# mikestir/webradio

Measured on AMD Instinct MI355X. Metric: complex Msamples/sec (node), 256-ch DDC+NFM demod, higher is better.
Workload: dtype f32

## Files before the change

### include/webradio_amd.h

```cpp
#ifndef WEBRADIO_AMD_H_
#define WEBRADIO_AMD_H_

#include <stddef.h>
#include <stdint.h>

#ifdef __cplusplus
extern "C" {
#endif

#define WR_ABI_VERSION   6
#define WR_FIR_LENGTH    64
#define WR_TABLE_SIZE    65536

enum wr_status {
	WR_OK = 0,
	WR_ERR_ARG = 1,
	WR_ERR_HIP = 2,
	WR_ERR_STATE = 3,
	WR_ERR_NOMEM = 4,
	WR_ERR_NODEV = 5,
	WR_ERR_RATE = 6
};

enum wr_mode { WR_AM = 0, WR_FM = 1, WR_USB = 2, WR_LSB = 3 };

enum wr_stage {
	WR_STAGE_CHAN_IQ = 1,
	WR_STAGE_DEMOD   = 2,
	WR_STAGE_AUDIO   = 3
};

enum wr_nco {
	WR_NCO_SPLIT = 0,
	WR_NCO_EXACT = 1,
	WR_NCO_ROTATE = 2
};

enum wr_where { WR_HOST = 0, WR_DEVICE = 1 };

typedef struct wr_dev      wr_dev;
typedef struct wr_tuner    wr_tuner;
typedef struct wr_spectrum wr_spectrum;
typedef struct wr_ring     wr_ring;

int         wr_abi_version(void);
const char *wr_last_error(void);
int         wr_device_count(int *count);
enum wr_tunable {
	WR_TUNE_DDC_NG2_MIN_PASSES = 1
};
int         wr_tune(int key, long value, long *previous);

int wr_phase_step(int if_hz, unsigned int input_rate, int *phase_step);
int wr_sin_table(float *table_host);
int wr_lowpass_design(unsigned int passband, unsigned int input_rate,
                      float *coeff_host , unsigned int *maxbin_out);
#define WR_FIR_MAX 1024
#define WR_FIR_FUSED_MAX 256
int wr_lowpass_design_n(unsigned int fir_length, unsigned int passband, unsigned int input_rate,
                        float *coeff_host , unsigned int *maxbin_out);
int wr_spectrum_window(unsigned int fft_size, float *window_host);

int wr_dev_open(wr_dev **dev, int device_index, void *hip_stream);
int wr_dev_close(wr_dev *dev);
int wr_dev_sync(wr_dev *dev);
void *wr_dev_stream(wr_dev *dev);
int wr_dev_malloc(wr_dev *dev, size_t bytes, void **ptr_dev);
int wr_dev_free(wr_dev *dev, void *ptr_dev);
int wr_dev_upload(wr_dev *dev, void *dst_dev, const void *src_host, size_t bytes);
int wr_dev_download(wr_dev *dev, void *dst_host, const void *src_dev, size_t bytes);
int wr_dev_host_register(wr_dev *dev, void *host, size_t bytes);
int wr_dev_host_unregister(wr_dev *dev, void *host);
int wr_dev_upload_async(wr_dev *dev, void *dst_dev, const void *src_host, size_t bytes);
int wr_dev_wait_uploads(wr_dev *dev);
int wr_dev_wait_uploads_but(wr_dev *dev, unsigned int newest);
int wr_dev_upload_ahead(wr_dev *dev, void *dst_dev, const void *src_host, size_t bytes);

int wr_mix(wr_dev *dev, const float *in_dev, float *out_dev, size_t nframes,
           unsigned int *phase_io, int phase_step);

int wr_fir_decimate(wr_dev *dev, const float *in_dev, size_t nframes, unsigned int channels,
                    unsigned int decimation, const float *coeff_host ,
                    float *history_dev, float *out_dev);
int wr_fir_decimate_n(wr_dev *dev, const float *in_dev, size_t nframes, unsigned int channels,
                      unsigned int decimation, unsigned int fir_length, const float *coeff_host ,
                      float *history_dev, float *out_dev);
unsigned long long wr_block_kernel_calls(void);

int wr_demod(wr_dev *dev, int mode, const float *in_dev, size_t nframes,
             float *prev_io , float *out_dev);

int wr_u8_to_f32(wr_dev *dev, const uint8_t *in_dev, float *out_dev, size_t count);
int wr_u8_to_f32_from_host(wr_dev *dev, const uint8_t *in_host_registered, float *out_dev, size_t count);
int wr_stage_windows_from_host(wr_dev *dev, const void *in_host_registered, int is_u8, float *out_dev, size_t nframes,
                               unsigned int period, unsigned int length, size_t tail_frames);

#define WR_MAX_CHANNELS 4096
int wr_tuner_create(wr_tuner **tuner, wr_dev *dev, unsigned int input_rate,
                    unsigned int max_channels, size_t max_block_frames, int nco_mode);
int wr_tuner_destroy(wr_tuner *tuner);

int wr_chan_add(wr_tuner *tuner, int *chan);
int wr_chan_remove(wr_tuner *tuner, int chan);
int wr_chan_count(wr_tuner *tuner, int *count);

int wr_chan_set_if(wr_tuner *tuner, int chan, int if_hz);
int wr_chan_set_filter(wr_tuner *tuner, int chan, int stage, unsigned int passband,
                       unsigned int out_rate);
int wr_chan_set_taps(wr_tuner *tuner, int chan, int stage, const float *coeff_host ,
                     unsigned int decimation);
int wr_chan_set_filter_n(wr_tuner *tuner, int chan, int stage, unsigned int fir_length,
                         unsigned int passband, unsigned int out_rate);
int wr_chan_set_taps_n(wr_tuner *tuner, int chan, int stage, const float *coeff_host ,
                       unsigned int fir_length, unsigned int decimation);
#define WR_FILTER_CHANNEL  0
#define WR_FILTER_AUDIO    1
#define WR_FILTER_CHANNEL2 2
int wr_chan_set_af_gain(wr_tuner *tuner, int chan, float gain_db);
int wr_chan_set_squelch(wr_tuner *tuner, int chan, float threshold_dbfs, int enable);
int wr_chan_set_mode(wr_tuner *tuner, int chan, int mode);
int wr_tuner_keep_stages(wr_tuner *tuner, unsigned int stage_mask);

int wr_chan_get_state(wr_tuner *tuner, int chan, unsigned int *phase, float *prev_iq );
int wr_chan_set_state(wr_tuner *tuner, int chan, unsigned int phase, const float *prev_iq);

int wr_tuner_last_staging(wr_tuner *tuner, int *how);
int wr_tuner_submit(wr_tuner *tuner, const float *iq, size_t nframes, int where);
int wr_tuner_submit_u8(wr_tuner *tuner, const uint8_t *iq_u8, size_t nframes, int where);

int wr_tuner_flush(wr_tuner *tuner);

int wr_chan_fetch(wr_tuner *tuner, int chan, int stage, float *out_host, size_t out_capacity,
                  size_t *count);
int wr_tuner_audio_dev(wr_tuner *tuner, const float **audio_dev, size_t *chan_stride,
                       size_t *frames);
int wr_chan_slot(wr_tuner *tuner, int chan, int *slot);
int wr_tuner_fetch_audio_all(wr_tuner *tuner, float *out_host, size_t out_capacity,
                             size_t *chan_stride, size_t *frames, unsigned int *slots_used);
int wr_tuner_audio_ring(wr_tuner *tuner, unsigned int depth);
int wr_tuner_audio_ring_acquire(wr_tuner *tuner, const float **audio_host, size_t *chan_stride,
                                size_t *frames, unsigned int *slots_used, unsigned long long *seq);
int wr_tuner_audio_ring_release(wr_tuner *tuner);
int wr_tuner_audio_ring_ready(wr_tuner *tuner, int *ready);
int wr_tuner_audio_ring_stats(wr_tuner *tuner, unsigned int *queued, unsigned long long *overruns);
int wr_tuner_submit_count(wr_tuner *tuner, unsigned long long *submits);
int wr_chan_reset_history(wr_tuner *tuner, int chan);
int wr_tuner_seek(wr_tuner *tuner, unsigned long long frame);
int wr_ring_id_bytes(void);
int wr_ring_version(int *version);
int wr_ring_make_id(void *id_host, size_t nbytes);
int wr_ring_create(wr_ring **ring, wr_dev *dev, const void *id_host, size_t nbytes, int rank, int world);
int wr_ring_exchange(wr_ring *ring, const float *send_dev, float *recv_dev, size_t nfloats);
int wr_tuner_mark_launches(wr_tuner *tuner, int enable);
int wr_ring_exchange_after(wr_ring *ring, wr_tuner *tuner, const float *send_dev, float *recv_dev, size_t nfloats);
int wr_ring_wait(wr_ring *ring);
int wr_ring_info(wr_ring *ring, int *rank, int *world, unsigned long long *exchanges);
int wr_ring_destroy(wr_ring *ring);
int wr_tuner_set_audio_scale(wr_tuner *tuner, float scale);

int wr_tuner_set_blocks_per_launch(wr_tuner *tuner, unsigned int nblocks);

#define WR_STREAM_MAX_BLOCKS 512u
int wr_tuner_set_streaming(wr_tuner *tuner, int enable);
int wr_tuner_stream_info(wr_tuner *tuner, int *live, unsigned long long *launches, unsigned long long *blocks);
int wr_tuner_stream_host_blocks(wr_tuner *tuner, unsigned long long *blocks);
int wr_tuner_stream_long_blocks(wr_tuner *tuner, unsigned long long *blocks);

int wr_tuner_profile(wr_tuner *tuner, int enable);
int wr_tuner_profile_read(wr_tuner *tuner, unsigned int *launches, double *mean_ms);

int wr_spectrum_create(wr_spectrum **spec, wr_dev *dev, unsigned int fft_size, unsigned int hop);
int wr_spectrum_destroy(wr_spectrum *spec);
int wr_spectrum_push(wr_spectrum *spec, const float *iq, size_t nframes, int where);
int wr_spectrum_lazy_info(wr_spectrum *spec, unsigned long long *deferred_pushes, unsigned long long *resolves);
int wr_spectrum_get_db(wr_spectrum *spec, float *magnitudes_host );
int wr_spectrum_get_bins(wr_spectrum *spec, float *bins_host );
int wr_spectrum_frames_done(wr_spectrum *spec, unsigned long *frames);
int wr_spectrum_get_waterfall_row(wr_spectrum *spec, unsigned int width, int hold,
                                  float *db_row_host, uint8_t *palette_host);
int wr_spectrum_batch_db(wr_spectrum *spec, const float *iq_dev, size_t nframes_fft,
                         float *db_dev);

#ifdef __cplusplus
}
#endif
#endif
```

### webradio_amd/capi.py

```python
import ctypes as C
import os

_HERE = os.path.dirname(os.path.abspath(__file__))
LIB_PATH = os.path.join(_HERE, "lib", "libwebradio_amd.so")

WR_OK, WR_ERR_ARG, WR_ERR_HIP, WR_ERR_STATE, WR_ERR_NOMEM, WR_ERR_NODEV, WR_ERR_RATE = range(7)
WR_AM, WR_FM, WR_USB, WR_LSB = range(4)
WR_STAGE_CHAN_IQ, WR_STAGE_DEMOD, WR_STAGE_AUDIO = 1, 2, 3
WR_NCO_SPLIT, WR_NCO_EXACT, WR_NCO_ROTATE = 0, 1, 2
WR_HOST, WR_DEVICE = 0, 1
WR_ABI_VERSION = 6
WR_STREAM_MAX_BLOCKS = 512
WR_FIR_LENGTH = 64
WR_TABLE_SIZE = 65536

_fp = C.POINTER(C.c_float)
_vp = C.c_void_p
_u32 = C.c_uint
_sz = C.c_size_t

SIGNATURES = {
    "wr_abi_version": (C.c_int, []),
    "wr_last_error": (C.c_char_p, []),
    "wr_device_count": (C.c_int, [C.POINTER(C.c_int)]),
    "wr_tune": (C.c_int, [C.c_int, C.c_long, C.POINTER(C.c_long)]),
    "wr_phase_step": (C.c_int, [C.c_int, _u32, C.POINTER(C.c_int)]),
    "wr_sin_table": (C.c_int, [_vp]),
    "wr_lowpass_design": (C.c_int, [_u32, _u32, _vp, C.POINTER(_u32)]),
    "wr_lowpass_design_n": (C.c_int, [_u32, _u32, _u32, _vp, C.POINTER(_u32)]),
    "wr_spectrum_window": (C.c_int, [_u32, _vp]),
    "wr_dev_open": (C.c_int, [C.POINTER(_vp), C.c_int, _vp]),
    "wr_dev_close": (C.c_int, [_vp]),
    "wr_dev_sync": (C.c_int, [_vp]),
    "wr_dev_stream": (_vp, [_vp]),
    "wr_dev_malloc": (C.c_int, [_vp, _sz, C.POINTER(_vp)]),
    "wr_dev_free": (C.c_int, [_vp, _vp]),
    "wr_dev_upload": (C.c_int, [_vp, _vp, _vp, _sz]),
    "wr_dev_download": (C.c_int, [_vp, _vp, _vp, _sz]),
    "wr_dev_host_register": (C.c_int, [_vp, _vp, _sz]),
    "wr_dev_host_unregister": (C.c_int, [_vp, _vp]),
    "wr_dev_upload_async": (C.c_int, [_vp, _vp, _vp, _sz]),
    "wr_dev_wait_uploads": (C.c_int, [_vp]),
    "wr_dev_wait_uploads_but": (C.c_int, [_vp, C.c_uint]),
    "wr_dev_upload_ahead": (C.c_int, [_vp, _vp, _vp, _sz]),
    "wr_mix": (C.c_int, [_vp, _vp, _vp, _sz, C.POINTER(_u32), C.c_int]),
    "wr_fir_decimate": (C.c_int, [_vp, _vp, _sz, _u32, _u32, _vp, _vp, _vp]),
    "wr_fir_decimate_n": (C.c_int, [_vp, _vp, _sz, _u32, _u32, _u32, _vp, _vp, _vp]),
    "wr_demod": (C.c_int, [_vp, C.c_int, _vp, _sz, _vp, _vp]),
    "wr_u8_to_f32": (C.c_int, [_vp, _vp, _vp, _sz]),
    "wr_stage_windows_from_host": (C.c_int, [_vp, _vp, C.c_int, _vp, _sz, _u32, _u32, _sz]),
    "wr_u8_to_f32_from_host": (C.c_int, [_vp, _vp, _vp, _sz]),
    "wr_tuner_create": (C.c_int, [C.POINTER(_vp), _vp, _u32, _u32, _sz, C.c_int]),
    "wr_tuner_destroy": (C.c_int, [_vp]),
    "wr_chan_add": (C.c_int, [_vp, C.POINTER(C.c_int)]),
    "wr_chan_remove": (C.c_int, [_vp, C.c_int]),
    "wr_chan_count": (C.c_int, [_vp, C.POINTER(C.c_int)]),
    "wr_chan_set_if": (C.c_int, [_vp, C.c_int, C.c_int]),
    "wr_chan_set_filter": (C.c_int, [_vp, C.c_int, C.c_int, _u32, _u32]),
    "wr_chan_set_taps": (C.c_int, [_vp, C.c_int, C.c_int, _vp, _u32]),
    "wr_chan_set_filter_n": (C.c_int, [_vp, C.c_int, C.c_int, _u32, _u32, _u32]),
    "wr_chan_set_taps_n": (C.c_int, [_vp, C.c_int, C.c_int, _vp, _u32, _u32]),
    "wr_chan_set_mode": (C.c_int, [_vp, C.c_int, C.c_int]),
    "wr_chan_set_af_gain": (C.c_int, [_vp, C.c_int, C.c_float]),
    "wr_chan_set_squelch": (C.c_int, [_vp, C.c_int, C.c_float, C.c_int]),
    "wr_tuner_keep_stages": (C.c_int, [_vp, _u32]),
    "wr_tuner_flush": (C.c_int, [_vp]),
    "wr_tuner_set_blocks_per_launch": (C.c_int, [_vp, _u32]),
    "wr_tuner_set_streaming": (C.c_int, [_vp, C.c_int]),
    "wr_tuner_stream_info": (C.c_int, [_vp, C.POINTER(C.c_int), C.POINTER(C.c_ulonglong), C.POINTER(C.c_ulonglong)]),
    "wr_tuner_stream_host_blocks": (C.c_int, [_vp, C.POINTER(C.c_ulonglong)]),
    "wr_tuner_stream_long_blocks": (C.c_int, [_vp, C.POINTER(C.c_ulonglong)]),
    "wr_tuner_seek": (C.c_int, [_vp, C.c_ulonglong]),
    "wr_tuner_audio_ring": (C.c_int, [_vp, _u32]),
    "wr_tuner_audio_ring_acquire": (C.c_int, [_vp, C.POINTER(C.POINTER(C.c_float)), C.POINTER(C.c_size_t),
                                              C.POINTER(C.c_size_t), C.POINTER(_u32), C.POINTER(C.c_ulonglong)]),
    "wr_tuner_audio_ring_release": (C.c_int, [_vp]),
    "wr_tuner_audio_ring_ready": (C.c_int, [_vp, C.POINTER(C.c_int)]),
    "wr_tuner_audio_ring_stats": (C.c_int, [_vp, C.POINTER(_u32), C.POINTER(C.c_ulonglong)]),
    "wr_tuner_submit_count": (C.c_int, [_vp, C.POINTER(C.c_ulonglong)]),
    "wr_chan_get_state": (C.c_int, [_vp, C.c_int, C.POINTER(_u32), _vp]),
    "wr_chan_set_state": (C.c_int, [_vp, C.c_int, _u32, _vp]),
    "wr_tuner_submit": (C.c_int, [_vp, _vp, _sz, C.c_int]),
    "wr_tuner_last_staging": (C.c_int, [_vp, C.POINTER(C.c_int)]),
    "wr_block_kernel_calls": (C.c_ulonglong, []),
    "wr_tuner_submit_u8": (C.c_int, [_vp, _vp, _sz, C.c_int]),
    "wr_chan_fetch": (C.c_int, [_vp, C.c_int, C.c_int, _vp, _sz, C.POINTER(_sz)]),
    "wr_tuner_audio_dev": (C.c_int, [_vp, C.POINTER(_vp), C.POINTER(_sz), C.POINTER(_sz)]),
    "wr_chan_slot": (C.c_int, [_vp, C.c_int, C.POINTER(C.c_int)]),
    "wr_tuner_fetch_audio_all": (C.c_int, [_vp, _vp, _sz, C.POINTER(_sz), C.POINTER(_sz), C.POINTER(_u32)]),
    "wr_chan_reset_history": (C.c_int, [_vp, C.c_int]),
    "wr_ring_id_bytes": (C.c_int, []),
    "wr_ring_version": (C.c_int, [C.POINTER(C.c_int)]),
    "wr_ring_make_id": (C.c_int, [_vp, _sz]),
    "wr_ring_create": (C.c_int, [C.POINTER(_vp), _vp, _vp, _sz, C.c_int, C.c_int]),
    "wr_ring_exchange": (C.c_int, [_vp, _vp, _vp, _sz]),
    "wr_ring_exchange_after": (C.c_int, [_vp, _vp, _vp, _vp, _sz]),
    "wr_tuner_mark_launches": (C.c_int, [_vp, C.c_int]),
    "wr_ring_wait": (C.c_int, [_vp]),
    "wr_ring_info": (C.c_int, [_vp, C.POINTER(C.c_int), C.POINTER(C.c_int), C.POINTER(C.c_ulonglong)]),
    "wr_ring_destroy": (C.c_int, [_vp]),
    "wr_tuner_set_audio_scale": (C.c_int, [_vp, C.c_float]),
    "wr_spectrum_get_waterfall_row": (C.c_int, [_vp, _u32, C.c_int, _vp, _vp]),
    "wr_tuner_profile": (C.c_int, [_vp, C.c_int]),
    "wr_tuner_profile_read": (C.c_int, [_vp, C.POINTER(_u32), C.POINTER(C.c_double)]),
    "wr_spectrum_create": (C.c_int, [C.POINTER(_vp), _vp, _u32, _u32]),
    "wr_spectrum_destroy": (C.c_int, [_vp]),
    "wr_spectrum_push": (C.c_int, [_vp, _vp, _sz, C.c_int]),
    "wr_spectrum_lazy_info": (C.c_int, [_vp, C.POINTER(C.c_ulonglong), C.POINTER(C.c_ulonglong)]),
    "wr_spectrum_get_db": (C.c_int, [_vp, _vp]),
    "wr_spectrum_get_bins": (C.c_int, [_vp, _vp]),
    "wr_spectrum_frames_done": (C.c_int, [_vp, C.POINTER(C.c_ulong)]),
    "wr_spectrum_batch_db": (C.c_int, [_vp, _vp, _sz, _vp]),
}


class WrError(RuntimeError):
    def __init__(self, code, msg):
        super().__init__("webradio_amd error %d: %s" % (code, msg))
        self.code = code


_lib = None


def load():
    global _lib
    if _lib is not None:
        return _lib
    if not os.path.exists(LIB_PATH):
        raise RuntimeError(
            "%s is missing: build it with `python -c 'import __graft_entry__ as g; g.build()'` "
            "(there is no CPU fallback)" % LIB_PATH)
    try:
        import torch
    except Exception:
        pass
    lib = C.CDLL(LIB_PATH, mode=C.RTLD_GLOBAL)
    for name, (res, args) in SIGNATURES.items():
        fn = getattr(lib, name)
        fn.restype = res
        fn.argtypes = args
    _lib = lib
    return lib


def check(rc):
    if rc != WR_OK:
        raise WrError(rc, load().wr_last_error().decode(errors="replace"))
    return rc


def ptr(x):
    if x is None:
        return None
    if isinstance(x, int):
        return C.c_void_p(x)
    if hasattr(x, "data_ptr"):
        return C.c_void_p(x.data_ptr())
    return C.c_void_p(x.ctypes.data)
```

### webradio_amd/csrc/wr_capi_internal.h

```cpp
#ifndef WR_CAPI_INTERNAL_H
#define WR_CAPI_INTERNAL_H

#include "wr_internal.h"

#include <cstdarg>
#include <cstdio>
#include <cstdlib>
#include <cstring>
#include <new>
#include <atomic>
#include <chrono>
#include <map>
#include <mutex>
#include <vector>

#define HIP_TRY(expr)                                                                    \
	do {                                                                                 \
		hipError_t e_ = (expr);                                                          \
		if (e_ != hipSuccess)                                                            \
			return wrc_fail(WR_ERR_HIP, "%s: %s (%s:%d)", #expr, hipGetErrorString(e_),  \
			                __FILE__, __LINE__);                                         \
	} while (0)


#define WR_UPLOAD_RING 4

struct wr_dev {
	int device;
	hipStream_t stream;
	bool own_stream;
	int num_cus;
	float *table;
	float *table_turn;
	float *turn_host;
	float *hi_cs, *lo_cs;
	float *scratch;
	size_t scratch_floats;
	float *coeff;
	std::mutex *scratch_lock;
	hipEvent_t upload_ev[WR_UPLOAD_RING];
	std::atomic<unsigned long long> uploads_issued, uploads_done;
	std::mutex *upload_lock;
	hipStream_t up_stream;
	hipStream_t lazy_stream = nullptr;
	hipEvent_t up_tail[WR_UPLOAD_RING], up_done;
	void *up_out[WR_UPLOAD_RING];
	unsigned long long up_calls;
	uint8_t *up_raw[2];
	size_t up_raw_cap[2];
	std::map<void *, size_t> *registered;
	wr_tuner *streaming = nullptr;
	unsigned long long reg_gen = 1;
};
#define SCRATCH_GUARD(d) std::lock_guard<std::mutex> scratch_guard_(*(d)->scratch_lock)

struct Chan {
	bool in_use;
	int if_hz;
	unsigned int stepL;
	unsigned int phaseL;
	int mode;
	bool have[3];
	float taps[3][WR_FIR_LENGTH];
	unsigned int len1;
	float taps_long[WR_FIR_FUSED_MAX];
	unsigned int len2, len1b;
	float taps_long2[WR_FIR_FUSED_MAX], taps_long1b[WR_FIR_FUSED_MAX];
	unsigned int decim[3];
	float gain;
	float squelch;
	bool cs_hist_reset;
	int group;
	int slot;
	float prev_iq[2];
	bool prev_dirty;
	bool phase_dirty;
	bool dem_hist_reset;
};

struct Group {
	unsigned int d1, d2;
	unsigned int d1b = 0;
	unsigned int l1 = WR_FIR_LENGTH;
	unsigned int l2 = WR_FIR_LENGTH;
	unsigned int l1b = WR_FIR_LENGTH;
	int p2 = 0;
	bool use_gain = false, use_squelch = false;
	unsigned int slots;
	size_t k1max, k2max;
	WrGroupDev dev;
	int audio_cur = 0;
	int parity;
	int last_parity;
	bool last_demod_kept = false;
	bool post_pending = false;
	WrPostArgs post_args;
	bool seek_pending = false;
	unsigned long long seek_frame = 0;
	float *z_hist = nullptr, *z_prev = nullptr, *z_dem = nullptr;
	bool pend_direct = false;
	unsigned long long pend_seq = 0;
	size_t pend_k2 = 0;
	unsigned int pend_slots = 0;
	int sp;
	int cb;
	int last_cb;
	std::vector<int> owner;
	bool dirty;
	bool uniform_taps;
	unsigned long long uniform_mask = 0;
	unsigned long long uniform2_mask = 0;
	unsigned long long fewsets_mask = 0;
	unsigned char nsets[64] = {0};
	bool one_filter = false;
	bool long_uniform = false;
	bool long_one = false;
	size_t last_k1, last_k2;
	int active;
};

struct wr_tuner {
	wr_dev *dev;
	unsigned int input_rate;
	unsigned int max_channels;
	size_t max_block_frames;
	int nco_mode;
	unsigned int keep_mask;
	std::vector<Chan> chans;
	std::vector<Group *> groups;
	float *in_stage;
	int last_staging = 0;
	const void *probe_ptr = nullptr;
	unsigned long long probe_gen = 0;
	unsigned int probe_left = 0;
	float *in_hist[2];
	int in_par;
	bool submitted;
	float audio_scale;
	bool profiling;
	unsigned int prof_stride;
	unsigned int prof_tick;
	std::vector<unsigned int> ev_span;
	bool mark_launches = false;
	hipEvent_t launch_ev[4] = {nullptr, nullptr, nullptr, nullptr};
	unsigned long long launches_marked = 0;
	std::vector<hipEvent_t> ev;
	size_t ev_used;
	double prof_ms;
	unsigned int prof_n;
	struct RingSlot {
		float *host = nullptr;
		size_t cap = 0;
		hipEvent_t done = nullptr;
		size_t stride = 0, frames = 0;
		unsigned int slots = 0;
		unsigned long long seq = 0;
		unsigned int stream_wait = 0;
		unsigned long long stream_gen = 0;
	};
	std::vector<RingSlot> ring;
	unsigned int ring_head = 0, ring_count = 0;
	bool ring_held = false;
	unsigned long long ring_overruns = 0;
	unsigned long long submit_seq = 0;
	bool defer_post = true;
	unsigned int coalesce = 1;
	const float *held_base = nullptr;
	size_t held_frames = 0, held_each = 0;
	unsigned int held_count = 0;
	std::mutex ring_lock;
	struct Stream {
		bool enabled = false;
		bool host_bytes = false;
		bool live = false;
		bool unchecked = false;
		WrStreamCtl *ctl = nullptr;
		WrStreamDesc *desc = nullptr;
		WrStreamDev *sdev = nullptr;
		float *ring = nullptr;
		size_t ring_floats = 0;
		Group *g = nullptr;
		unsigned int count = 0;
		size_t nframes = 0;
		bool u8 = false;
		int parity0 = 0;
		size_t k1 = 0, k2 = 0;
		unsigned long long gen = 0;
		unsigned long long blocks = 0;
		std::chrono::steady_clock::time_point last_bell;
		const float *last_iq = nullptr;
		uint8_t *raw[4] = {nullptr, nullptr, nullptr, nullptr};
		size_t raw_cap = 0;
		unsigned long long raw_next = 0;
		unsigned long long raw_gen[4] = {0, 0, 0, 0};
		unsigned int raw_idx[4] = {0, 0, 0, 0};
		hipEvent_t raw_ev = nullptr;
		bool ext = false;
		bool up_pending = false;
		unsigned long long host_blocks = 0;
		unsigned long long long_blocks = 0;
	} stream;
};

struct wr_spectrum {
	wr_dev *dev;
	unsigned int n, hop;
	WrFftPlan plan;
	float *stage;
	size_t stage_cap;
	size_t pending;
	float *bins;
	unsigned long frames_done;
	bool deferred = false;
	float *keep_host = nullptr;
	size_t keep_cap = 0;
	size_t def_off = 0, def_keep = 0;
	size_t def_rest = 0;
	hipEvent_t def_ev = nullptr;
	unsigned long long deferred_pushes = 0, resolves = 0;
};


int        wrc_dev_bind(wr_dev *d);
int        wrc_dev_settle_stream(wr_dev *d);
hipError_t wrc_dev_stream_sync(wr_dev *d);
int        wrc_dev_scratch(wr_dev *d, size_t floats);
void      *wrc_host_mapped(const void *host, hipError_t *why = nullptr);
int        wrc_upload_mark_locked(wr_dev *d, hipStream_t st);
int        wrc_upload_mark(wr_dev *d, hipStream_t st);
int        wrc_dev_up_stream(wr_dev *d);

unsigned int  wrc_group_slots_used(const Group *g);
WrTunerLaunch wrc_group_launch(const wr_tuner *t, const Group *g, const float *cur, const uint8_t *cur_u8, size_t nframes);
Group        *wrc_single_group(wr_tuner *t, bool *several = nullptr);
int           wrc_group_upload(wr_tuner *t, Group *g);
int           wrc_settle_held(wr_tuner *t);
int           wrc_tuner_launch_held(wr_tuner *t);
int           wrc_tuner_flush(wr_tuner *t);
int           wrc_tuner_quiesce(wr_tuner *t);
int           wrc_tuner_submit_now(wr_tuner *t, const void *iq, size_t nframes, int where, bool u8);
void          wrc_advance_phases(wr_tuner *t, unsigned long long frames);
int           wrc_prof_pair_begin(wr_tuner *t, void **ev_start, void **ev_stop);
void          wrc_prof_pair_stamped(wr_tuner *t);

int  wrc_stream_close(wr_tuner *t);
int  wrc_stream_check(wr_tuner *t);
void wrc_stream_free(wr_tuner *t);
bool wrc_stream_follows(const wr_tuner *t, size_t nframes, int where, bool u8);
int  wrc_stream_bell(wr_tuner *t, const void *iq, bool behind_upload);
int  wrc_stream_open(wr_tuner *t, const void *iq, size_t nframes, bool u8, bool *took);
int  wrc_stream_host_u8(wr_tuner *t, const uint8_t *bytes, size_t nframes, bool *took);

float *wrc_ring_reserve(wr_tuner *t, Group *g, size_t k2, unsigned int used);
int    wrc_ring_push(wr_tuner *t, Group *g, unsigned long long seq, size_t k2, unsigned int used, bool direct);
float *wrc_stream_ring_entry(wr_tuner *t, Group *g, unsigned long long seq, size_t k2, unsigned int used, unsigned int idx);

#define DEV_SETTLE(d_) do { if (int rc_ = wrc_dev_settle_stream(d_)) return rc_; } while (0)
#define TUNER_SYNC_CHECKED(t_) do { HIP_TRY(wrc_dev_stream_sync((t_)->dev)); if (int rc_ = wrc_stream_check(t_)) return rc_; } while (0)

#define WR_STREAM_IDLE_MS   500
#define WR_STREAM_STALE_MS  100
#define WR_STREAM_WAIT_MS  2000
#define WR_STREAM_HOST_MIN_BYTES (16u << 10)

#endif
```

### webradio_amd/csrc/wr_internal.h

```cpp
#ifndef WR_INTERNAL_H_
#define WR_INTERNAL_H_

#include <hip/hip_runtime.h>
#include <stddef.h>
#include <stdint.h>

#include "webradio_amd.h"

#define WR_HIST      (WR_FIR_LENGTH - 1)
#define WR_LANES     64
#define WR_SPLIT_N   256
#define WR_MAX_DEVICES 64
#define WR_TAPSETS   4

int         wrc_fail(int code, const char *fmt, ...) __attribute__((format(printf, 2, 3)));
int         wrc_dev_index(const wr_dev *dev);
hipStream_t wrc_dev_stream(const wr_dev *dev);
int         wrc_tuner_launch_mark(wr_tuner *t, hipEvent_t *ev);

void     wrd_sin_table(float *table);
void     wrd_sin_table_rounded(float *table);
int      wrd_phase_step(int if_hz, unsigned int input_rate);
unsigned wrd_lowpass_maxbin(unsigned int fir_length, unsigned int passband, unsigned int input_rate);
void     wrd_lowpass_design(unsigned int fir_length, unsigned int passband, unsigned int input_rate, float *coeff);
void     wrd_spectrum_window(unsigned int n, float *window);
void     wrd_split_tables(float *hi_cs , float *lo_cs );
void     wrd_twiddles(unsigned int n, float *tw );

struct WrGroupDev {
	unsigned int *phase[2];
	unsigned int *step;
	float        *hist_cs[2];
	float        *hist_lo[2];
	int          *flags;
	int          *mode;
	float        *taps1;
	float        *taps2;
	float        *taps2u;
	float        *rot;
	float        *taps1u;
	int          *tapsel;
	float        *taps1b;
	float        *iq2_hist[2];
	float        *chan_iq2[2];
	float        *taps1L;
	float        *mixhist[2];
	float        *gain;
	float        *squelch;
	float        *prev_iq[2];
	float        *chan_iq[2];
	float        *dem[2];
	float        *audio;
	float        *audio_set[4];
	unsigned int  l2 = 64, l1b = 64;
};

struct WrTunerLaunch {
	const float *cur;
	const uint8_t *cur_u8;
	const float *hist;
	float       *hist_next;
	int          parity;
	int          sp;
	int          cb;
	size_t       nframes;
	unsigned int d1, d2;
	unsigned int slots;
	unsigned int slots_used;
	size_t       k1, k2;
	size_t       k2max;
	int          nco_mode;
	float        audio_scale;
	int          use_gain, use_squelch;
	unsigned long long uniform_mask;
	unsigned long long uniform2_mask;
	unsigned long long fewsets_mask;
	unsigned char nsets[64];
	int          one_filter;
	void        *ev_start, *ev_stop;
	bool         seeking = false;
	unsigned int seek_lo = 0;
};

hipError_t wrk_mix(hipStream_t st, const float *in, float *out, size_t nframes,
                   unsigned int phase, int step, const float *table_dev);
hipError_t wrk_fir(hipStream_t st, const float *in, size_t nframes, unsigned int channels,
                   unsigned int decim, unsigned int fir_length, const float *coeff_dev, const float *hist_dev,
                   float *out);
hipError_t wrk_hist_update(hipStream_t st, const float *in, size_t nframes, unsigned int channels,
                           unsigned int fir_length, float *hist_dev, float *scratch_dev);
hipError_t wrk_demod(hipStream_t st, int mode, const float *in, size_t nframes, float prev_i,
                     float prev_q, float *out);
hipError_t wrk_u8_to_f32(hipStream_t st, const uint8_t *in, float *out, size_t count);
hipError_t wrk_stage_windows(hipStream_t st, const void *src_mapped, bool u8, float *dst, size_t nframes, unsigned int period,
                             unsigned int len, size_t tail_frames);

struct WrPostArgs {
	const float *chan_iq;
	unsigned int k1, slots;
	const int   *mode;
	const float *prev_iq;
	float       *prev_next;
	const float *dem_hist;
	float       *dem_hist_next;
	size_t       k2;
	unsigned int tiles;
	unsigned int run;
	unsigned int ntiles;
	const float *taps2;
	const float *taps2u;
	unsigned long long uni2;
	float       *audio;
	size_t       k2max;
	float        scale;
	unsigned int d2;
	unsigned int groups;
	const float *gain;
	const float *squelch;
	float       *audio_host;
	size_t       host_stride;
	unsigned int nseg = 1;
	const float *chan_prev = nullptr;
};
long wrk_tune_ng2_min_passes(long value, bool set);
hipError_t wrk_tuner_ddc(hipStream_t st, const WrTunerLaunch &L, const WrGroupDev &G,
                         const float *table_dev, const float *hi_dev, const float *lo_dev,
                         int num_cus, const WrPostArgs *post = nullptr, bool *post_taken = nullptr);
hipError_t wrk_tuner_ddc_long(hipStream_t st, const WrTunerLaunch &L, const WrGroupDev &G, unsigned int len,
                              const float *table_dev, int num_cus, bool rotate, bool rotate_one_filter, const float *hi_dev,
                              const float *lo_dev, const WrPostArgs *post = nullptr, bool *post_taken = nullptr);
hipError_t wrk_tuner_demod(hipStream_t st, const WrTunerLaunch &L, const WrGroupDev &G);
hipError_t wrk_tuner_iq2(hipStream_t st, const WrGroupDev &G, unsigned int slots, unsigned int slots_used,
                         size_t k1a, unsigned int d1b, int cb, int p2);
hipError_t wrk_tuner_audio(hipStream_t st, const WrTunerLaunch &L, const WrGroupDev &G);
WrPostArgs wrk_post_args(const WrTunerLaunch &L, const WrGroupDev &G);
hipError_t wrk_tuner_post(hipStream_t st, const WrTunerLaunch &L, const WrGroupDev &G);
hipError_t wrk_tuner_post_args(hipStream_t st, const WrPostArgs &A);
bool wrk_tuner_post_supported(unsigned int d2);
hipError_t wrk_input_hist(hipStream_t st, const float *cur, const uint8_t *cur_u8, size_t nframes,
                          const float *hist, float *hist_next);
hipError_t wrk_seek(hipStream_t st, const WrGroupDev &G, unsigned int slots, int sp, int parity, int p2,
                    unsigned long long frame);
hipError_t wrk_gather_rows(hipStream_t st, const float *src, size_t rows, size_t row_stride_floats,
                           size_t col_offset_floats, unsigned int width_floats, float *dst);

#define WR_STREAM_MAXJ   WR_STREAM_MAX_BLOCKS
#define WR_STREAM_RING   6u
struct WrStreamDesc {
	unsigned long long cur;
	unsigned long long audio_host;
	unsigned int count;
	unsigned int pad;
};
struct WrStreamCtl {
	volatile unsigned int ready;
	volatile unsigned int stop;
	volatile unsigned int pad0[14];
	volatile unsigned int done;
	volatile unsigned int final_blocks;
	volatile unsigned int err;
	volatile unsigned int self_closed;
	volatile unsigned int long_blocks;
	volatile unsigned int pad1[11];
};
#define WR_STREAM_SHARDS 16u
struct WrStreamDev {
	unsigned int ready, stop;
	unsigned long long beat;
	unsigned int ready_up;
	unsigned int pad0[27];
	unsigned long long progress;
	unsigned int drain_from;
	unsigned int pad1[29];
	unsigned int post_done[WR_STREAM_MAXJ];
	unsigned int post_fine[WR_STREAM_MAXJ];
	unsigned int post_ticket[WR_STREAM_MAXJ];
	unsigned int ddc_done[WR_STREAM_MAXJ][WR_STREAM_SHARDS][32];
	WrStreamDesc desc[WR_STREAM_MAXJ];
	unsigned long long cur[WR_STREAM_MAXJ + 1u];
};
struct WrStreamArgs {
	WrStreamCtl        *ctl;
	const WrStreamDesc *desc_host;
	WrStreamDev        *sdev;
	unsigned long long  idle_ticks;
	unsigned long long  wait_ticks;
	unsigned int        n_ddc, n_post;
	unsigned long long *tl;
	unsigned long long  cur0, audio0;
	unsigned long long  nframes;
	unsigned int        k1, d1, is_u8;
	unsigned int        ext;
	unsigned int        slots, groups;
	unsigned long long  gmap0, gmap1;
	unsigned int        kslow;
	unsigned int        kmax;
	const float        *hist;
	float              *hist_next;
	const unsigned int *phase, *step;
	unsigned int       *phase_next;
	const float        *hist_cs, *hist_lo;
	float              *hist_cs_next, *hist_lo_next;
	const int          *flags;
	const float        *taps1, *rot, *taps1u;
	const int          *tapsel;
	const float        *table, *hi_cs, *lo_cs;
	float              *ring;
	float              *audio_bufs[4];
	WrPostArgs          post;
	unsigned int        drain_run, drain_ntiles;
	const float        *prev_iq[2];
	float              *dem[2];
	int                 parity0;
	unsigned int        one_filter;
};
#define WR_STREAM_ERR_WAIT   1u
hipError_t wrk_stream_geometry(unsigned int d2, unsigned int groups, unsigned int kmax, bool one_filter, unsigned int nseg,
                               int num_cus, unsigned int *n_ddc, unsigned int *n_post);
hipError_t wrk_tuner_stream(hipStream_t st, const WrStreamArgs &A, void *ev_start, void *ev_stop);

struct WrFftPlan {
	unsigned int n;
	unsigned int n1, n2;
	float *tw_n;
	float *tw_sub;
	float *window;
	float *window_p1;
	float *work;
	size_t work_frames;
};
hipError_t wrk_fft_frames(hipStream_t st, const WrFftPlan &P, const float *iq, size_t hop,
                          size_t nframes_fft, float *bins_out , float *db_out );

hipError_t wrk_bins_to_db(hipStream_t st, const float *bins, unsigned int n, float *db);
hipError_t wrk_waterfall_row(hipStream_t st, const float *bins, unsigned int n, unsigned int width, int hold,
                             float *db_row, uint8_t *palette);

#endif
```

### webradio_amd/csrc/wr_kernels.hip

```cpp
#include "wr_internal.h"

#include <atomic>
#include <cstdlib>
#include <type_traits>

#include <hip/hip_ext.h>

typedef float v2f __attribute__((ext_vector_type(2)));
typedef __attribute__((address_space(3))) v2f lds_v2f;
typedef float v4f __attribute__((ext_vector_type(4)));
typedef __attribute__((address_space(3))) v4f lds_v4f;

#define PHASE_FLAG_ACTIVE   1

#define WR_CONSTANT __attribute__((address_space(4)))

#ifdef DDC_TIMELINE
#define TL_SLOTS 12
__device__ unsigned long long g_ddc_tl[16384 * TL_SLOTS];
extern "C" int wr_debug_timeline(unsigned long long *out, size_t n)
{
	return (int)hipMemcpyFromSymbol(out, HIP_SYMBOL(g_ddc_tl), n * sizeof(unsigned long long));
}
__device__ unsigned long long g_ddc_rt[16384 * 2];
// ... 49 lines not shown
		out[n] = y;
	}
}

__global__ void __launch_bounds__(256)
k_fir(const float *__restrict__ in, size_t outfloats, unsigned int channels, unsigned int decim,
      unsigned int L, const float *__restrict__ coeff, const float *__restrict__ hist, float *__restrict__ out)
{
	__shared__ float taps[WR_FIR_MAX];
	for (unsigned int j = threadIdx.x; j < L; j += blockDim.x)
		taps[j] = coeff[j];
	__syncthreads();
	const unsigned int nh = L - 1u;
	size_t stride = (size_t)gridDim.x * blockDim.x;
	for (size_t o = (size_t)blockIdx.x * blockDim.x + threadIdx.x; o < outfloats; o += stride) {
		size_t k = o / channels;
		unsigned int c = (unsigned int)(o - k * channels);
		size_t first = k * decim;
		float acc = 0.0f;
		for (unsigned int j = 0; j < L; ++j) {
			size_t f = first + j;
			float x = (f < nh) ? hist[f * channels + c] : in[(f - nh) * channels + c];
			acc = acc + taps[L - 1u - j] * x;
		}
		out[o] = acc;
	}
}

__global__ void k_hist_build(const float *__restrict__ in, size_t nframes, unsigned int channels, unsigned int nh,
                             const float *__restrict__ hist, float *__restrict__ scratch)
{
	unsigned int total = nh * channels;
	for (unsigned int e = blockIdx.x * blockDim.x + threadIdx.x; e < total; e += gridDim.x * blockDim.x) {
		size_t f = nframes + e / channels;
		unsigned int c = e % channels;
		scratch[e] = (f < nh) ? hist[f * channels + c] : in[(f - nh) * channels + c];
	}
}

__global__ void k_copy_f32(const float *__restrict__ src, float *__restrict__ dst, size_t n)
{
	size_t stride = (size_t)gridDim.x * blockDim.x;
	for (size_t i = (size_t)blockIdx.x * blockDim.x + threadIdx.x; i < n; i += stride)
		dst[i] = src[i];
}

__device__ __forceinline__ float fm_angle_cycles(float y, float x)
{
	const float ax = __builtin_fabsf(x), ay = __builtin_fabsf(y);
	const float mx = __builtin_fmaxf(ax, ay), mn = __builtin_fminf(ax, ay);
	const float sc = (mx < 0x1p-100f) ? 0x1p100f : 1.0f;
	const float r = (mx == 0.0f) ? 0.0f : (mn * sc) * __builtin_amdgcn_rcpf(mx * sc);
	const float t = r * r;
	float p = 0.002456712769344449f;
	p = __builtin_fmaf(p, t, -0.014401308260858059f);
	p = __builtin_fmaf(p, t, 0.03978113830089569f);
	p = __builtin_fmaf(p, t, -0.07234849780797958f);
	p = __builtin_fmaf(p, t, 0.1049894168972969f);
	p = __builtin_fmaf(p, t, -0.14161227643489838f);
	p = __builtin_fmaf(p, t, 0.19985906779766083f);
	p = __builtin_fmaf(p, t, -0.33332598209381104f);
	p = __builtin_fmaf(p, t, 0.9999998807907104f);
	float c = (p * r) * 0.15915494309189533577f;
	if (ay > ax)
		c = 0.25f - c;
	if (__builtin_signbitf(x))
		c = 0.5f - c;
	return __builtin_copysignf(c, y);
}

__device__ __forceinline__ float demod_one(int mode, float i, float q, float pi_, float pq_)
{
	switch (mode) {
	case WR_AM:
		return (float)sqrt((double)(i * i + q * q));
	case WR_FM: {
		float ii = i * pi_ + q * pq_;
		float qq = q * pi_ - i * pq_;
		return fm_angle_cycles(ii, qq);
	}
	case WR_USB:
		return i + q;
	default:
		return i - q;
	}
}

__global__ void __launch_bounds__(256)
k_demod(int mode, const float2 *__restrict__ in, size_t nframes, float prev_i, float prev_q,
        float *__restrict__ out)
{
	size_t stride = (size_t)gridDim.x * blockDim.x;
	for (size_t n = (size_t)blockIdx.x * blockDim.x + threadIdx.x; n < nframes; n += stride) {
		float2 z = in[n];
		float2 p = n ? in[n - 1] : make_float2(prev_i, prev_q);
		out[n] = demod_one(mode, z.x, z.y, p.x, p.y);
	}
}

__global__ void k_u8_to_f32(const uint8_t *__restrict__ in, float *__restrict__ out, size_t n)
{
	size_t stride = (size_t)gridDim.x * blockDim.x;
	for (size_t i = (size_t)blockIdx.x * blockDim.x + threadIdx.x; i < n; i += stride)
		out[i] = ((float)in[i] - 128.0f) / 128.0f;
}

#define U8_X16_WGS 128u
__global__ void __launch_bounds__(256) k_u8_to_f32_x16(const uint4 *__restrict__ in, float4 *__restrict__ out, size_t n16)
{
	const size_t stride = (size_t)gridDim.x * blockDim.x;
	for (size_t i0 = (size_t)blockIdx.x * blockDim.x + threadIdx.x; i0 < n16; i0 += 4 * stride) {
		uint4 v[4];
#pragma unroll
		for (int u = 0; u < 4; ++u)
			if (i0 + u * stride < n16)
				v[u] = in[i0 + u * stride];
#pragma unroll
		for (int u = 0; u < 4; ++u) {
			const size_t i = i0 + u * stride;
			if (i >= n16)
				break;
			const unsigned int w[4] = {v[u].x, v[u].y, v[u].z, v[u].w};
#pragma unroll
			for (int q = 0; q < 4; ++q) {
				float4 o;
				o.x = ((float)(w[q] & 255u) - 128.0f) / 128.0f;
				o.y = ((float)((w[q] >> 8) & 255u) - 128.0f) / 128.0f;
				o.z = ((float)((w[q] >> 16) & 255u) - 128.0f) / 128.0f;
				o.w = ((float)(w[q] >> 24) - 128.0f) / 128.0f;
				out[4 * i + q] = o;
			}
		}
	}
}


template <int NCO>
__device__ __forceinline__ v2f nco(unsigned int P, const float *__restrict__ table,
                                   const v2f *hi_l, const v2f *lo_l)
{
	if (NCO == WR_NCO_EXACT) {
		v2f cs;
		cs.y = table[P >> 16];
		cs.x = table[(P + 0x40000000u) >> 16];
		return cs;
	} else {
		constexpr unsigned int SH = (NCO == WR_NCO_SPLIT) ? 5u : 0u;
		const v2f a = hi_l[(P >> 24) << SH];
		const v2f b = lo_l[((P >> 16) & 255u) << SH];
		const v2f rot = {-a.y, a.x};
		return __builtin_elementwise_fma(rot, b.yy, a * b.xx);
	}
}

template <int NCO>
__device__ __forceinline__ void mac(v2f xs, v2f cs, float hj, v2f &acc)
{
	if (NCO == WR_NCO_EXACT) {
		const float mi = xs.x * cs.x + xs.y * cs.y;
		const float mq = xs.y * cs.x - xs.x * cs.y;
		float ti, tq;
		asm("v_mul_f32 %0, %1, %2" : "=v"(ti) : "v"(hj), "v"(mi));
		asm("v_mul_f32 %0, %1, %2" : "=v"(tq) : "v"(hj), "v"(mq));
		acc.x = acc.x + ti;
		acc.y = acc.y + tq;
	} else {
		const v2f xr = {xs.y, -xs.x};
		const v2f m = __builtin_elementwise_fma(xr, cs.yy, xs * cs.xx);
		asm("v_fmac_f32 %0, %1, %2" : "+v"(acc.x) : "v"(hj), "v"(m.x));
		asm("v_fmac_f32 %0, %1, %2" : "+v"(acc.y) : "v"(hj), "v"(m.y));
	}
}

__device__ __forceinline__ unsigned int rot_index(unsigned int p0, unsigned int st, unsigned int m)
{
	const unsigned int P = p0 + m * st;
	return (st >> 16) + (((P & 0xFFFFu) < (st & 0xFFFFu)) ? 1u : 0u);
}

__device__ __forceinline__ v2f rot_into(unsigned int p0, unsigned int st, unsigned int m,
                                        const float *__restrict__ table)
{
	const unsigned int idx = rot_index(p0, st, m);
	v2f r;
	r.y = table[idx & 0xFFFFu];
	r.x = table[(idx + 16384u) & 0xFFFFu];
	return r;
}

__device__ __forceinline__ void horner_step(v2f &A, float rc, float rs, v2f u)
{
	const float tr = __builtin_fmaf(-A.y, rs, u.x);
	const float ti = __builtin_fmaf(A.x, rs, u.y);
	const float ar = __builtin_fmaf(A.x, rc, tr);
	const float ai = __builtin_fmaf(A.y, rc, ti);
	A.x = ar;
	A.y = ai;
}

__device__ __forceinline__ void horner_close(v2f &y, v2f A, v2f cs)
{
	const float yr = __builtin_fmaf(A.y, cs.y, __builtin_fmaf(A.x, cs.x, y.x));
	const float yi = __builtin_fmaf(-A.x, cs.y, __builtin_fmaf(A.y, cs.x, y.y));
	y.x = yr;
	y.y = yi;
}

__device__ __forceinline__ void wave_prio(unsigned int level)
{
	if (level >= 3u)
		__builtin_amdgcn_s_setprio(3);
	else if (level == 2u)
		__builtin_amdgcn_s_setprio(2);
	else if (level == 1u)
		__builtin_amdgcn_s_setprio(1);
	else
		__builtin_amdgcn_s_setprio(0);
}

__device__ __forceinline__ void rot_tables_to_lds(v2f *lds, const float2 *hi_cs, const float2 *lo_cs)
{
	for (unsigned int e = threadIdx.x; e < WR_SPLIT_N; e += blockDim.x) {
		const float2 hv = hi_cs[e], lv = lo_cs[e];
		lds[e] = (v2f){hv.x, hv.y};
		lds[WR_SPLIT_N + e] = (v2f){lv.x, lv.y};
	}
	__syncthreads();
}

#define ROT_SEG 64
#define ROT_Q   (WR_FIR_LENGTH / ROT_SEG)
#define SLOW_CH 4

__device__ __forceinline__ void gather_split(unsigned int P, unsigned int &ah, unsigned int &al,
                                             v2f &a, v2f &b)
{
	asm("v_mov_b32_sdwa %0, %1 dst_sel:BYTE_1 dst_unused:UNUSED_PRESERVE src0_sel:BYTE_3"
	    : "+v"(ah) : "v"(P));
	asm("v_mov_b32_sdwa %0, %1 dst_sel:BYTE_1 dst_unused:UNUSED_PRESERVE src0_sel:BYTE_2"
	    : "+v"(al) : "v"(P));
	a = *(const lds_v2f *)(uintptr_t)ah;
	b = *(const lds_v2f *)(uintptr_t)al;
}

__device__ __forceinline__ float2 input_frame(const float2 *__restrict__ cur, const uchar2 *__restrict__ cur_u8,
                                              size_t n)
{
	if (cur_u8) {
		const uchar2 b = cur_u8[n];
		return make_float2(((float)b.x - 128.0f) / 128.0f, ((float)b.y - 128.0f) / 128.0f);
	}
	return cur[n];
}

#define POST_TK 16u
#define POST_B 4u
#define POST_LB 5u
#define POST_THREADS 512u
__device__ __forceinline__ float audio_out(float v, const float *__restrict__ gain, const float *__restrict__ squelch,
                                           const float2 *__restrict__ chan_iq, unsigned int slots, unsigned int so,
                                           size_t k, unsigned int d2, float scale)
{
	if (squelch) {
		const float thr = squelch[so];
		if (thr > 0.0f) {
			float p = 0.0f;
			for (unsigned int i = 0; i < d2; ++i) {
				const float2 z = chan_iq[(k * d2 + i) * slots + so];
				p = p + (z.x * z.x + z.y * z.y);
			}
			if (p / (float)d2 < thr)
				v = 0.0f;
		}
	}
	if (gain) {
		const float gn = gain[so];
		if (gn != 1.0f)
			v = v * gn;
	}
	return (scale == 1.0f) ? v : v * scale;
}

__device__ __forceinline__ float post_row(const float2 *__restrict__ chan_iq, unsigned int k1, unsigned int slots,
                                          unsigned int s, int m, const float2 *__restrict__ prev_iq,
                                          const float *__restrict__ dem_hist, size_t rr,
                                          const float2 *__restrict__ chan_prev = nullptr, unsigned int hist = WR_HIST)
{
	if (rr < hist) {
		if (!chan_prev)
			return dem_hist[rr * slots + s];
		const size_t kp = (size_t)k1 - hist + rr;
		const float2 z = chan_prev[kp * slots + s];
		const float2 zp = chan_prev[(kp - 1u) * slots + s];
		return demod_one(m, z.x, z.y, zp.x, zp.y);
	}
	const size_t kk = rr - hist;
	if (kk >= k1)
		return 0.0f;
	const float2 z = chan_iq[kk * slots + s];
	const float2 zp = kk ? chan_iq[(kk - 1u) * slots + s] : chan_prev ? chan_prev[((size_t)k1 - 1u) * slots + s] : prev_iq[s];
	return demod_one(m, z.x, z.y, zp.x, zp.y);
}

template <unsigned int D2, bool HREGS, unsigned int NSEG = 1u>
__device__ __forceinline__ void post_role(const WrPostArgs &A, unsigned int bx, unsigned int g,
                                          float *stage, float *tile, int *modes)
{
	constexpr unsigned int HIST = WR_FIR_LENGTH * NSEG - 1u;
	constexpr unsigned int NEED = (POST_TK - 1u) * D2 + WR_FIR_LENGTH * NSEG;
	constexpr unsigned int NROW = POST_THREADS / 64u;
	static_assert(NSEG == 1u || !HREGS, "the segmented filter reads its taps when their turn comes (measured at C2, 128 / 256 taps: "
	                                    "61 / 83 us per block; a segment's 64 taps fetched into registers first: 64 / 94)");
	const float2 *__restrict__ chan_iq = (const float2 *)A.chan_iq;
	const float2 *__restrict__ prev_iq = (const float2 *)A.prev_iq;
	const float2 *__restrict__ chan_prev = (const float2 *)A.chan_prev;
	const float *__restrict__ dem_hist = A.dem_hist;
	const float *__restrict__ taps2 = A.taps2;
	const unsigned int k1 = A.k1, slots = A.slots;
	const unsigned int lane = threadIdx.x & 63u;
	const unsigned int row = threadIdx.x >> 6;
	const unsigned int s = g * 64u + lane;
	const int m = A.mode[s];

	if (bx == A.ntiles) {
		if (m < 0)
			return;
		const size_t first = k1;
#pragma unroll
		for (unsigned int r = row; r < HIST; r += NROW)
			A.dem_hist_next[(size_t)r * slots + s] = post_row(chan_iq, k1, slots, s, m, prev_iq, dem_hist, first + r, chan_prev, HIST);
		if (row == 0)
			((float2 *)A.prev_next)[s] = k1 ? chan_iq[(size_t)(k1 - 1u) * slots + s] : prev_iq[s];
		return;
	}

	TLP(0);
	float h[HREGS ? WR_FIR_LENGTH : 1];
	if (HREGS && row < POST_TK / POST_B) {
#pragma unroll
		for (int j = 0; j < (HREGS ? WR_FIR_LENGTH : 1); ++j)
			h[j] = taps2[(size_t)j * slots + s];
	}
	if (row == 0)
		modes[lane] = m;
	constexpr unsigned int FRESH = POST_TK * D2;
	constexpr unsigned int CARRY = NEED - FRESH;
	constexpr unsigned int CARRY_PER = (CARRY * 64u + POST_THREADS - 1u) / POST_THREADS;
	for (unsigned int tt = 0; tt < A.run; ++tt) {
		const unsigned int tl = bx * A.run + tt;
		if (tl >= A.tiles)
			break;
		const size_t kbase = (size_t)tl * POST_TK;
		const size_t r0 = kbase * D2;
		unsigned int first = 0;
		if (tt) {
			float keep[CARRY_PER];
#pragma unroll
			for (unsigned int i = 0; i < CARRY_PER; ++i) {
				const unsigned int e = threadIdx.x + i * POST_THREADS;
				keep[i] = (e < CARRY * 64u) ? stage[FRESH * 64u + e] : 0.0f;
			}
			__syncthreads();
#pragma unroll
			for (unsigned int i = 0; i < CARRY_PER; ++i) {
				const unsigned int e = threadIdx.x + i * POST_THREADS;
				if (e < CARRY * 64u)
					stage[e] = keep[i];
			}
			first = CARRY;
		}
		{
			const unsigned int per = (NEED - first + NROW - 1u) / NROW;
			const unsigned int beg = first + row * per;
			const unsigned int end = (beg + per < NEED) ? beg + per : NEED;
			if (r0 > HIST && r0 + NEED <= (size_t)k1 + HIST) {
				const float2 *__restrict__ src = chan_iq + (r0 - HIST) * slots + s;
				for (unsigned int r = beg; r < end; r += POST_LB) {
					float2 z[POST_LB + 1u];
					z[0] = src[((size_t)r - 1u) * slots];
#pragma unroll
					for (unsigned int i = 0; i < POST_LB; ++i) {
						const unsigned int ri = (r + i < end) ? r + i : end - 1u;
						z[i + 1u] = src[(size_t)ri * slots];
					}
#pragma unroll
					for (unsigned int i = 0; i < POST_LB; ++i)
						if (r + i < end)
							stage[(r + i) * 64u + lane] = (m >= 0) ? demod_one(m, z[i + 1u].x, z[i + 1u].y, z[i].x, z[i].y) : 0.0f;
				}
			} else {
				float2 zp = make_float2(0.0f, 0.0f);
				if (m >= 0 && beg < end) {
					const size_t rr = r0 + beg;
					if (rr == HIST)
						zp = chan_prev ? chan_prev[((size_t)k1 - 1u) * slots + s] : prev_iq[s];
					else if (rr > HIST && rr - HIST - 1u < k1)
						zp = chan_iq[(rr - HIST - 1u) * slots + s];
					else if (rr < HIST && chan_prev)
						zp = chan_prev[((size_t)k1 - HIST - 1u + rr) * slots + s];
				}
#pragma unroll 6
				for (unsigned int r = beg; r < end; ++r) {
					const size_t rr = r0 + r;
					float v = 0.0f;
					if (m >= 0) {
						if (rr < HIST && chan_prev) {
							const float2 z = chan_prev[((size_t)k1 - HIST + rr) * slots + s];
							v = demod_one(m, z.x, z.y, zp.x, zp.y);
							zp = z;
						} else if (rr < HIST) {
							v = dem_hist[rr * slots + s];
							if (rr + 1u == HIST)
								zp = prev_iq[s];
						} else if (rr - HIST < k1) {
							const float2 z = chan_iq[(rr - HIST) * slots + s];
							v = demod_one(m, z.x, z.y, zp.x, zp.y);
							zp = z;
						}
					}
					stage[r * 64u + lane] = v;
				}
			}
		}
		__syncthreads();
		TLP(1);
		if (row < POST_TK / POST_B) {
			float acc[POST_B];
#pragma unroll
			for (unsigned int o = 0; o < POST_B; ++o)
				acc[o] = 0.0f;
			if (HREGS) {
				const float *x = stage + (row * POST_B * D2) * 64u + lane;
#pragma unroll
				for (unsigned int r = 0; r < (POST_B - 1u) * D2 + WR_FIR_LENGTH; ++r) {
					const float xv = x[r * 64u];
#pragma unroll
					for (unsigned int o = 0; o < POST_B; ++o) {
						if (r >= o * D2 && r - o * D2 < WR_FIR_LENGTH)
							acc[o] = acc[o] + h[HREGS ? WR_FIR_LENGTH - 1u - (r - o * D2) : 0] * xv;
					}
				}
			} else {
#pragma unroll 1
			for (unsigned int seg = 0; seg < NSEG; ++seg) {
				const float *x = stage + (row * POST_B * D2 + seg * WR_FIR_LENGTH) * 64u + lane;
				const unsigned int tap0 = (NSEG - 1u - seg) * WR_FIR_LENGTH;
				if (g < 64u && ((A.uni2 >> g) & 1ull)) {
					const WR_CONSTANT float *tu = (const WR_CONSTANT float *)(A.taps2u + (size_t)g * (WR_FIR_LENGTH * NSEG) + tap0);
#pragma unroll
					for (int j = WR_FIR_LENGTH - 1; j >= 0; --j) {
						const float hj = tu[j];
#pragma unroll
						for (unsigned int o = 0; o < POST_B; ++o)
							acc[o] = acc[o] + hj * x[(o * D2 + (WR_FIR_LENGTH - 1u - (unsigned int)j)) * 64u];
					}
				} else {
#pragma unroll 16
					for (int j = WR_FIR_LENGTH - 1; j >= 0; --j) {
						const float hj = taps2[((size_t)tap0 + j) * slots + s];
#pragma unroll
						for (unsigned int o = 0; o < POST_B; ++o)
							acc[o] = acc[o] + hj * x[(o * D2 + (WR_FIR_LENGTH - 1u - (unsigned int)j)) * 64u];
					}
				}
			}
			}
#pragma unroll
			for (unsigned int o = 0; o < POST_B; ++o)
				tile[(row * POST_B + o) * 65u + lane] = acc[o];
		}
		__syncthreads();
		TLP(2);
		for (unsigned int e = threadIdx.x; e < 64u * POST_TK; e += POST_THREADS) {
			const unsigned int sl = e / POST_TK, kk = e - sl * POST_TK;
			const unsigned int so = g * 64u + sl;
			const size_t k = kbase + kk;
			if (k < A.k2 && modes[sl] >= 0) {
				const float v = audio_out(tile[kk * 65u + sl], A.gain, A.squelch, chan_iq, slots, so, k, D2, A.scale);
				A.audio[(size_t)so * A.k2max + k] = v;
				if (A.audio_host)
					A.audio_host[(size_t)so * A.host_stride + k] = v;
			} else if (k < A.k2 && A.audio_host) {
				A.audio_host[(size_t)so * A.host_stride + k] = 0.0f;
			}
		}
		TLP(3);
	}
}

template <unsigned int D2, unsigned int NSEG = 1u>
__global__ void __launch_bounds__(POST_THREADS)
k_tuner_post(WrPostArgs A)
{
	constexpr unsigned int NEED = (POST_TK - 1u) * D2 + WR_FIR_LENGTH * NSEG;
	if constexpr (NSEG == 1u) {
		__shared__ float stage[NEED * 64u];
		__shared__ float tile[POST_TK * 65u];
		__shared__ int modes[64];
		post_role<D2, NSEG == 1u, NSEG>(A, blockIdx.x, blockIdx.y, stage, tile, modes);
	} else {
		extern __shared__ float post_lds[];
		float *stage = post_lds;
		float *tile = stage + NEED * 64u;
		int *modes = (int *)(tile + POST_TK * 65u);
		post_role<D2, NSEG == 1u, NSEG>(A, blockIdx.x, blockIdx.y, stage, tile, modes);
	}
}

#define DDC_TABLE_BYTES   (2u * WR_SPLIT_N * 32u * 8u)
#define DDC_WAVES         16u
#define DDC_ROTATE_WAVES      8u
#define DDC_ROTATE_WGS_PER_CU 4u
#define DDC_LDS_BYTES     (DDC_TABLE_BYTES + DDC_WAVES * 2u * 512u)
#define DDC_DEAL_WAYS 2u

#define DDC_PARAMS \
	const float2 *__restrict__ cur, const uchar2 *__restrict__ cur_u8, const float2 *__restrict__ hist, \
	float2 *__restrict__ hist_next, size_t nframes, size_t k1, unsigned int d1, unsigned int slots, unsigned int groups, \
	const unsigned int *__restrict__ phase, const unsigned int *__restrict__ step, \
	const float2 *__restrict__ hist_cs, const int *__restrict__ flags, \
	unsigned int *__restrict__ phase_next, float2 *__restrict__ hist_cs_next, \
	const float2 *__restrict__ hist_lo, float2 *__restrict__ hist_lo_next, \
	const float *__restrict__ taps1, const float4 *__restrict__ rot, const float *__restrict__ taps1u, \
	const int *__restrict__ tapsel, unsigned int kmax, float2 *__restrict__ chan_iq, \
	const float *__restrict__ table, const float2 *__restrict__ hi_cs, const float2 *__restrict__ lo_cs, \
	unsigned int n_ddc, const WrPostArgs &post, unsigned long long gmap0, unsigned long long gmap1, int whole, \
	unsigned int kslow, unsigned int n_bnd, unsigned int seek_on, unsigned int seek_lo
#define DDC_PASS \
	cur, cur_u8, hist, hist_next, nframes, k1, d1, slots, groups, phase, step, hist_cs, flags, phase_next, hist_cs_next, \
	hist_lo, hist_lo_next, taps1, rot, taps1u, tapsel, kmax, chan_iq, table, hi_cs, lo_cs, n_ddc, post, gmap0, gmap1, \
	whole, kslow, n_bnd, seek_on, seek_lo
#define DDC_PHASE(s_) (seek_on ? step[s_] * seek_lo : phase[s_])
#define DDC_ROLE_ALL      0
#define DDC_ROLE_BOUNDARY 1
#define DDC_ROLE_ROLL     2

template <int NCO, bool UTAPS, unsigned int PD2>
__device__ __forceinline__ void
ddc_body(DDC_PARAMS, v2f *lds, const int role)
{
	if (PD2 != 0u && role != DDC_ROLE_ROLL && blockIdx.x >= n_ddc + n_bnd) {
		wave_prio(3u);
		constexpr unsigned int NEED = (POST_TK - 1u) * (PD2 ? PD2 : 1u) + WR_FIR_LENGTH;
		const unsigned int idx = blockIdx.x - n_ddc - n_bnd;
		if (threadIdx.x >= POST_THREADS)
			return;
		float *stage = (float *)lds;
		post_role<(PD2 ? PD2 : 1u), false>(post, idx % (post.ntiles + 1u), idx / (post.ntiles + 1u), stage,
		                                    stage + NEED * 64u, (int *)(stage + NEED * 64u + POST_TK * 65u));
		return;
	}
	const unsigned int lane = threadIdx.x & 63u;
	const unsigned int wave = __builtin_amdgcn_readfirstlane(threadIdx.x >> 6);
	const unsigned int waves_per_wg = blockDim.x >> 6;
	const unsigned int wid = blockIdx.x * waves_per_wg + wave;
	TL(0);
	wave_prio(3u);

	if (NCO == WR_NCO_SPLIT) {
		for (unsigned int e = threadIdx.x; e < WR_SPLIT_N * 32u; e += blockDim.x) {
			const float2 hv = hi_cs[e >> 5], lv = lo_cs[e >> 5];
			lds[e] = (v2f){hv.x, hv.y};
			lds[WR_SPLIT_N * 32u + e] = (v2f){lv.x, lv.y};
		}
		__syncthreads();
	} else if (NCO == WR_NCO_ROTATE) {
		rot_tables_to_lds(lds, hi_cs, lo_cs);
	}
	const v2f *hi_l = (NCO == WR_NCO_ROTATE) ? lds : lds + (lane & 31u);
	const v2f *lo_l = (NCO == WR_NCO_ROTATE) ? lds + WR_SPLIT_N : lds + WR_SPLIT_N * 32u + (lane & 31u);
	const unsigned int a_hi = (unsigned int)(uintptr_t)hi_l;
	const unsigned int a_lo = (unsigned int)(uintptr_t)lo_l;
	const unsigned int nset = UTAPS ? kmax : 1u;
	v2f *win = lds + (NCO == WR_NCO_SPLIT ? DDC_TABLE_BYTES / 8u : NCO == WR_NCO_ROTATE ? 2u * WR_SPLIT_N : 0u)
	           + wave * (128u * nset);

	if (whole && role != DDC_ROLE_ROLL && blockIdx.x == 0 && wave == 0 && lane < WR_HIST) {
		const size_t f = nframes + lane;
		hist_next[lane] = (f < WR_HIST) ? hist[f] : input_frame(cur, cur_u8, f - WR_HIST);
	}

	const unsigned int k1u = (unsigned int)k1;
	const unsigned int nwaves = n_ddc * waves_per_wg;
	TL(1);
	constexpr bool LTAPS = (NCO == WR_NCO_ROTATE) && !UTAPS;
	unsigned int wpg = LTAPS ? (n_ddc / groups) * waves_per_wg : nwaves / groups;
	const bool bnd = role == DDC_ROLE_BOUNDARY;
	const unsigned int ub = bnd ? (blockIdx.x - n_ddc) * waves_per_wg + wave : 0u;
	const unsigned int gl = bnd ? ub % groups : LTAPS ? blockIdx.x % groups : wid % groups;
	const unsigned int g = (unsigned int)(((gl < 8u ? gmap0 : gmap1) >> ((gl & 7u) * 8u)) & 255u);
	unsigned int k = bnd ? ub / groups : LTAPS ? (blockIdx.x / groups) * waves_per_wg + wave : wid / groups;
	if (role == DDC_ROLE_ROLL) {
		k = k1u;
	} else if (bnd) {
		if (k >= kslow)
			k = k1u;
		wpg = k1u;
	} else if (k >= wpg) {
		k = k1u;
	} else if (!LTAPS) {
		const unsigned int r = k % DDC_DEAL_WAYS, q = k / DDC_DEAL_WAYS;
		const unsigned int fl_ = wpg / DDC_DEAL_WAYS, rem = wpg % DDC_DEAL_WAYS;
		k = r * fl_ + (r < rem ? r : rem) + q;
	}
	const float *ltaps = (const float *)(lds + (NCO == WR_NCO_ROTATE ? 2u * WR_SPLIT_N : 0u) + waves_per_wg * 128u * nset);
	if (LTAPS) {
		float *lt = (float *)(lds + 2u * WR_SPLIT_N + waves_per_wg * 128u * nset);
		for (unsigned int e = threadIdx.x; e < WR_FIR_LENGTH * 64u; e += blockDim.x)
			lt[e] = taps1[(size_t)(e >> 6) * slots + g * 64u + (e & 63u)];
		__syncthreads();
	}

	float h[(UTAPS || LTAPS) ? 1 : WR_FIR_LENGTH];
	float hlane[UTAPS ? WR_TAPSETS : 1];
	unsigned int mysel = 0;
#pragma unroll
	for (int q = 0; q < (UTAPS ? WR_TAPSETS : 1); ++q)
		hlane[q] = 0.0f;
	unsigned int p0 = 0, st = 0;
	int fl = 0;
	unsigned int buf = 0;
	v2f rot0 = {1.0f, 0.0f}, rot1 = {1.0f, 0.0f};

	auto window_sample = [&](unsigned int kk) -> float2 {
		const long long n = (long long)kk * d1 - WR_HIST + lane;
		return (n >= 0) ? input_frame(cur, cur_u8, (size_t)n) : hist[WR_HIST + n];
	};
	float2 xnext = make_float2(0.0f, 0.0f);
	float2 xnext2 = make_float2(0.0f, 0.0f);
	const unsigned int s = g * 64u + lane;
	if (k < k1u) {
		{
			p0 = DDC_PHASE(s);
			st = step[s];
			fl = flags[s];
			if (NCO == WR_NCO_ROTATE) {
				const float4 r = rot[s];
				rot0 = (v2f){r.x, r.y};
				rot1 = (v2f){r.z, r.w};
			}
			if (UTAPS) {
				mysel = (unsigned int)tapsel[s];
#pragma unroll
				for (int q = 0; q < (UTAPS ? WR_TAPSETS : 1); ++q)
					if ((unsigned int)q < nset)
						hlane[q] = taps1u[((size_t)g * WR_TAPSETS + q) * 64u + lane];
			} else {
#pragma unroll
				for (int j = 0; j < ((UTAPS || LTAPS) ? 1 : WR_FIR_LENGTH); ++j)
					h[j] = taps1[(size_t)j * slots + s];
			}
		}
		xnext = window_sample(k);
		if (k + wpg < k1u)
			xnext2 = window_sample(k + wpg);
	}

	TL(2);
	unsigned int tl_unit = 0;
	const unsigned int my_units = (k < k1u) ? (k1u - k + wpg - 1u) / wpg : 0u;
	for (; k < k1u; buf ^= 1u) {
		const unsigned int kn = k + wpg;
		{
			const unsigned int q = (4u * tl_unit) / (my_units ? my_units : 1u);
			wave_prio(q >= 3u ? 0u : 2u - q + 0u);
		}

		const long long n0 = (long long)k * d1 - WR_HIST;
		{
			const float2 xf = xnext;
			if (UTAPS) {
#pragma unroll
				for (int q = 0; q < (UTAPS ? WR_TAPSETS : 1); ++q)
					if ((unsigned int)q < nset)
						win[(buf * nset + q) * 64u + lane] = (v2f){hlane[q] * xf.x, hlane[q] * xf.y};
			} else {
				win[buf * 64u + lane] = (v2f){xf.x, xf.y};
			}
// ... 1634 lines not shown
```

### webradio_amd/csrc/wr_stream_kernel.inc

```

__device__ __forceinline__ unsigned int st_rfl(unsigned int v) { return __builtin_amdgcn_readfirstlane(v); }
__device__ __forceinline__ unsigned int st_ld(const unsigned int *p)
{
	return st_rfl(__hip_atomic_load(p, __ATOMIC_RELAXED, __HIP_MEMORY_SCOPE_AGENT));
}
__device__ __forceinline__ unsigned long long st_ld64(const unsigned long long *p)
{
	const unsigned long long v = __hip_atomic_load(p, __ATOMIC_RELAXED, __HIP_MEMORY_SCOPE_AGENT);
	return ((unsigned long long)st_rfl((unsigned int)(v >> 32)) << 32) | st_rfl((unsigned int)v);
}
__device__ __forceinline__ unsigned int st_ld_sys(const volatile unsigned int *p)
{
	return st_rfl(__hip_atomic_load((const unsigned int *)p, __ATOMIC_RELAXED, __HIP_MEMORY_SCOPE_SYSTEM));
}
__device__ __forceinline__ void st_st_sys(volatile unsigned int *p, unsigned int v)
{
	__hip_atomic_store((unsigned int *)p, v, __ATOMIC_RELAXED, __HIP_MEMORY_SCOPE_SYSTEM);
}

__device__ __forceinline__ unsigned int st_ddc_ready(const WrStreamArgs &S)
{
	return st_rfl((unsigned int)__hip_atomic_load(&S.sdev->progress, __ATOMIC_RELAXED, __HIP_MEMORY_SCOPE_AGENT));
}
__device__ __forceinline__ unsigned int st_post_ready(const WrStreamArgs &S)
{
	return st_rfl((unsigned int)(__hip_atomic_load(&S.sdev->progress, __ATOMIC_RELAXED, __HIP_MEMORY_SCOPE_AGENT) >> 32));
}

__device__ __forceinline__ void stream_fail(const WrStreamArgs &S)
{
	st_st_sys(&S.ctl->err, WR_STREAM_ERR_WAIT);
	__hip_atomic_store(&S.sdev->stop, 1u, __ATOMIC_RELAXED, __HIP_MEMORY_SCOPE_AGENT);
}

__device__ __forceinline__ bool stream_wait_ready(const WrStreamArgs &S, unsigned int need, unsigned int &known, bool &closed)
{
	if (need < known)
		return true;
	if (closed)
		return false;
	const unsigned long long t0 = __builtin_amdgcn_s_memrealtime();
	unsigned int spins = 0;
	for (;;) {
		const unsigned int r = st_ld(&S.sdev->ready);
		if (r > need) {
			known = r;
			return true;
		}
		if (st_ld(&S.sdev->stop)) {
			const unsigned int f = st_ld(&S.sdev->ready);
			if (f > known)
				known = f;
			closed = true;
			return known > need;
		}
		if ((++spins & 63u) == 0u) {
			const unsigned long long now = __builtin_amdgcn_s_memrealtime();
			const unsigned long long beat = __hip_atomic_load(&S.sdev->beat, __ATOMIC_RELAXED, __HIP_MEMORY_SCOPE_AGENT);
			if (now - t0 > S.wait_ticks && now >= beat && now - beat > S.wait_ticks) {
				stream_fail(S);
				if (r > known)
					known = r;
				closed = true;
				return false;
			}
		}
		__builtin_amdgcn_s_sleep(20);
	}
}

__device__ __forceinline__ bool stream_wait_count(const WrStreamArgs &S, const unsigned int *p, unsigned int target)
{
	if (st_ld(p) >= target)
		return true;
	const unsigned long long t0 = __builtin_amdgcn_s_memrealtime();
	unsigned int spins = 0;
	for (;;) {
		__builtin_amdgcn_s_sleep(20);
		if (st_ld(p) >= target)
			return true;
		if ((++spins & 63u) == 0u) {
			if (__builtin_amdgcn_s_memrealtime() - t0 > S.wait_ticks) {
				stream_fail(S);
				return false;
			}
			if (st_ld_sys(&S.ctl->err))
				return false;
		}
	}
}

#define STREAM_DRAIN_BLOCKS 2u
__device__ __forceinline__ void stream_watch(const WrStreamArgs &S)
{
	const unsigned int lane = threadIdx.x & 63u;
	__builtin_amdgcn_s_setprio(3);
	const unsigned int units = S.k1 * S.groups;
	unsigned int known = 1, jd = 0, jp = 0;
	unsigned int df = 0;
	unsigned int nlong = 0;
	bool closed = false;
	unsigned long long t_last = __builtin_amdgcn_s_memrealtime();
#ifdef STREAM_TL
	if ((threadIdx.x & 63u) == 0 && S.tl)
		S.tl[6999u * 8u + 0u] = t_last;
#endif
	for (;;) {
		bool moved = false;
		auto look = [&]() __attribute__((always_inline)) {
			const unsigned int r = st_ld(&S.sdev->ready);
			if (r > known)
				known = r;
			if (st_ld(&S.sdev->stop)) {
				const unsigned int f = st_ld(&S.sdev->ready);
				if (f > known)
					known = f;
				closed = true;
				const unsigned int from = known >= STREAM_DRAIN_BLOCKS ? known - STREAM_DRAIN_BLOCKS : 0u;
				df = (jd > from ? jd : from) + 1u;
				__hip_atomic_store(&S.sdev->drain_from, df, __ATOMIC_RELAXED, __HIP_MEMORY_SCOPE_AGENT);
				__builtin_amdgcn_fence(__ATOMIC_RELEASE, "agent");
			}
		};
		if (!closed && (jd >= known || jp >= known))
			look();
		if (jd < known && jd < WR_STREAM_MAXJ) {
			unsigned int v = 0;
			if (lane < WR_STREAM_SHARDS)
				v = __hip_atomic_load(&S.sdev->ddc_done[jd][lane][0], __ATOMIC_RELAXED, __HIP_MEMORY_SCOPE_AGENT);
#pragma unroll
			for (int o = 8; o >= 1; o >>= 1)
				v += __shfl_xor(v, o, 64);
			if (st_rfl(v) >= units) {
				{
					unsigned int fine = 1u;
					if (S.drain_run != S.post.run) {
						if (!closed)
							look();
						fine = (df && jd + 1u >= df) ? 1u : known >= jd + 3u ? 0u : 1u;
					}
					__hip_atomic_store(&S.sdev->post_fine[jd], fine, __ATOMIC_RELAXED, __HIP_MEMORY_SCOPE_AGENT);
					if (!fine && lane == 0)
						st_st_sys(&S.ctl->long_blocks, ++nlong);
					asm volatile("s_waitcnt vmcnt(0)" ::: "memory");
				}
				++jd;
				__hip_atomic_store(&S.sdev->progress, ((unsigned long long)jp << 32) | jd, __ATOMIC_RELAXED, __HIP_MEMORY_SCOPE_AGENT);
				moved = true;
#ifdef STREAM_TL
				if (lane == 0 && S.tl && jd <= 256u)
					S.tl[(7000u + jd - 1u) * 8u + 0u] = __builtin_amdgcn_s_memrealtime();
#endif
			}
		}
		if (jp < jd && st_ld(&S.sdev->post_done[jp]) >= (st_ld(&S.sdev->post_fine[jp]) ? S.drain_ntiles : S.post.ntiles) * S.post.groups) {
			++jp;
			__hip_atomic_store(&S.sdev->progress, ((unsigned long long)jp << 32) | jd, __ATOMIC_RELAXED, __HIP_MEMORY_SCOPE_AGENT);
			if (lane == 0)
				st_st_sys(&S.ctl->done, jp);
			moved = true;
#ifdef STREAM_TL
			if (lane == 0 && S.tl && jp <= 256u)
				S.tl[(7000u + jp - 1u) * 8u + 1u] = __builtin_amdgcn_s_memrealtime();
#endif
		}
		if (closed && jp >= known)
			return;
		const unsigned long long now = __builtin_amdgcn_s_memrealtime();
		if (moved) {
			t_last = now;
		} else {
			if ((jd < known || jp < jd) && now - t_last > S.wait_ticks) {
				stream_fail(S);
				return;
			}
			if (closed && st_ld_sys(&S.ctl->err))
				return;
			__builtin_amdgcn_s_sleep(4);
		}
	}
}

__device__ __forceinline__ void stream_bell(const WrStreamArgs &S)
{
	if (threadIdx.x >= 64u && threadIdx.x < 128u) {
		stream_watch(S);
		return;
	}
	if (threadIdx.x != 0)
		return;
	__builtin_amdgcn_s_setprio(3);
	unsigned int seen = 1;
	__hip_atomic_store(&S.sdev->desc[0].cur, S.cur0, __ATOMIC_RELAXED, __HIP_MEMORY_SCOPE_AGENT);
	__hip_atomic_store(&S.sdev->desc[0].audio_host, S.audio0, __ATOMIC_RELAXED, __HIP_MEMORY_SCOPE_AGENT);
	__hip_atomic_store(&S.sdev->cur[1], S.cur0, __ATOMIC_RELAXED, __HIP_MEMORY_SCOPE_AGENT);
	asm volatile("s_waitcnt vmcnt(0)" ::: "memory");
	unsigned long long t_last = __builtin_amdgcn_s_memrealtime();
	for (;;) {
		__hip_atomic_store(&S.sdev->beat, (unsigned long long)__builtin_amdgcn_s_memrealtime(), __ATOMIC_RELAXED,
		                   __HIP_MEMORY_SCOPE_AGENT);
		const unsigned int s = st_ld_sys(&S.ctl->stop);
		unsigned int r = st_ld_sys(&S.ctl->ready);
		{
			const unsigned int ru = st_ld(&S.sdev->ready_up);
			if (ru > r)
				r = ru;
		}
		if (r > WR_STREAM_MAXJ)
			r = WR_STREAM_MAXJ;
		if (r > seen) {
			for (unsigned int j = seen; j < r; ++j) {
				const unsigned long long c = __hip_atomic_load(&S.desc_host[j].cur, __ATOMIC_RELAXED, __HIP_MEMORY_SCOPE_SYSTEM);
				const unsigned long long a = __hip_atomic_load(&S.desc_host[j].audio_host, __ATOMIC_RELAXED, __HIP_MEMORY_SCOPE_SYSTEM);
				__hip_atomic_store(&S.sdev->desc[j].cur, c, __ATOMIC_RELAXED, __HIP_MEMORY_SCOPE_AGENT);
				__hip_atomic_store(&S.sdev->cur[j + 1u], c, __ATOMIC_RELAXED, __HIP_MEMORY_SCOPE_AGENT);
				__hip_atomic_store(&S.sdev->desc[j].audio_host, a, __ATOMIC_RELAXED, __HIP_MEMORY_SCOPE_AGENT);
			}
			asm volatile("s_waitcnt vmcnt(0)" ::: "memory");
			__hip_atomic_store(&S.sdev->ready, r, __ATOMIC_RELAXED, __HIP_MEMORY_SCOPE_AGENT);
			seen = r;
			t_last = __builtin_amdgcn_s_memrealtime();
		}
		if (s || st_ld(&S.sdev->stop)) {
			asm volatile("s_waitcnt vmcnt(0)" ::: "memory");
			__hip_atomic_store(&S.sdev->stop, 1u, __ATOMIC_RELAXED, __HIP_MEMORY_SCOPE_AGENT);
			return;
		}
		if (seen >= WR_STREAM_MAXJ || __builtin_amdgcn_s_memrealtime() - t_last > S.idle_ticks) {
			if (seen < WR_STREAM_MAXJ)
				st_st_sys(&S.ctl->self_closed, 1u);
			asm volatile("s_waitcnt vmcnt(0)" ::: "memory");
			__hip_atomic_store(&S.sdev->stop, 1u, __ATOMIC_RELAXED, __HIP_MEMORY_SCOPE_AGENT);
			return;
		}
		__builtin_amdgcn_s_sleep(40);
	}
}

template <unsigned int PD2, unsigned int TS, unsigned int NSEG>
__device__ __forceinline__ void stream_post(const WrStreamArgs &S, const unsigned int p, v2f *lds, const bool helper)
{
	constexpr unsigned int D2 = PD2 ? PD2 : 1u;
	constexpr unsigned int NEED = (POST_TK - 1u) * D2 + WR_FIR_LENGTH * NSEG;
	wave_prio(3u);
	if (threadIdx.x >= POST_THREADS)
		return;
	const unsigned int wave = st_rfl(threadIdx.x >> 6);
	const unsigned int waves_per_wg = POST_THREADS / 64u;
#ifdef STREAM_TL
	if (threadIdx.x == 0 && S.tl && !helper)
		S.tl[(6000u + p) * 8u + 7u] = 12345ull;
#endif

	const unsigned int n_bnd = (S.kslow * S.groups + waves_per_wg - 1u) / waves_per_wg;
	if (!helper && p < n_bnd) {
		const unsigned long long c0 = S.cur0;
		ddc_body<WR_NCO_ROTATE, true, PD2>(S.is_u8 ? nullptr : (const float2 *)c0, S.is_u8 ? (const uchar2 *)c0 : nullptr,
		                                   (const float2 *)S.hist, (float2 *)S.hist_next, (size_t)S.nframes, (size_t)S.k1, S.d1,
		                                   S.slots, S.groups, S.phase, S.step, (const float2 *)S.hist_cs, S.flags, S.phase_next,
		                                   (float2 *)S.hist_cs_next, (const float2 *)S.hist_lo, (float2 *)S.hist_lo_next, S.taps1,
		                                   (const float4 *)S.rot, S.taps1u, S.tapsel, TS == 1u ? 1u : S.kmax, (float2 *)S.ring, S.table,
		                                   (const float2 *)S.hi_cs, (const float2 *)S.lo_cs, S.n_ddc, S.post, S.gmap0, S.gmap1, 0,
		                                   S.kslow, 0x40000000u, 0u, 0u, lds, DDC_ROLE_BOUNDARY);
		const unsigned int ub = p * waves_per_wg + wave;
		asm volatile("s_waitcnt vmcnt(0)" ::: "memory");
		if (ub / S.groups < S.kslow && (threadIdx.x & 63u) == 0u)
			__hip_atomic_fetch_add(&S.sdev->ddc_done[0][ub % WR_STREAM_SHARDS][0], 1u, __ATOMIC_RELAXED, __HIP_MEMORY_SCOPE_AGENT);
		wave_prio(3u);
		__syncthreads();
	}

	float *stage = (float *)lds;
	float *tile = stage + NEED * 64u;
	int *modes = (int *)(tile + POST_TK * 65u);
	unsigned int *sh = (unsigned int *)(modes + 64);
	const unsigned int tasks = S.post.ntiles * S.post.groups;
	unsigned int known = 1;
	bool closed = false;
	unsigned int j = 0;
	if (helper) {
		if (threadIdx.x == 0)
			sh[6] = st_ld(&S.sdev->drain_from);
		__syncthreads();
		const unsigned int df = sh[6];
		if (!df)
			return;
		j = df - 1u;
	}
#ifdef STREAM_TL
	unsigned long long pt_wait = 0, pt_work = 0, pt_sync = 0, pt_n = 0;
#endif
	for (;; ++j) {
#ifdef STREAM_TL
		const unsigned long long pt0 = __builtin_amdgcn_s_memtime();
#endif
		if (threadIdx.x == 0) {
			bool ok = j < WR_STREAM_MAXJ && stream_wait_ready(S, j, known, closed);
			if (ok) {
				const unsigned int need_hi = j >= 4u ? j - 3u : 0u;
				const unsigned long long t0 = __builtin_amdgcn_s_memrealtime();
				unsigned int spins = 0;
				for (;;) {
					const unsigned long long pg = st_ld64(&S.sdev->progress);
					if ((unsigned int)pg >= j + 1u && (unsigned int)(pg >> 32) >= need_hi)
						break;
					if ((++spins & 63u) == 0u) {
						if (__builtin_amdgcn_s_memrealtime() - t0 > S.wait_ticks) {
							stream_fail(S);
							ok = false;
							break;
						}
						if (st_ld_sys(&S.ctl->err)) {
							ok = false;
							break;
						}
					}
					__builtin_amdgcn_s_sleep(20);
				}
			}
			unsigned long long ah = 0;
			unsigned int drain = helper ? 1u : 0u;
			if (ok) {
				ah = j ? st_ld64(&S.sdev->desc[j].audio_host) : S.audio0;
				__builtin_amdgcn_fence(__ATOMIC_ACQUIRE, "agent");
				if (!helper) {
					const unsigned int df = st_ld(&S.sdev->drain_from);
					drain = (df && j + 1u >= df) ? 1u : 0u;
				}
				sh[7] = (helper || drain) ? 1u : st_ld(&S.sdev->post_fine[j]);
			}
			sh[5] = drain;
			sh[0] = ok ? 1u : 0u;
			sh[1] = (unsigned int)ah;
			sh[2] = (unsigned int)(ah >> 32);
			sh[3] = known;
		}
		__syncthreads();
		const bool go = sh[0] != 0u;
		const unsigned long long ah = ((unsigned long long)sh[2] << 32) | sh[1];
		known = sh[3];
		if (!go)
			break;
		WrPostArgs A = S.post;
		A.chan_iq = S.ring + (size_t)(j % WR_STREAM_RING) * S.k1 * S.slots * 2u;
		A.chan_prev = j ? S.ring + (size_t)((j - 1u) % WR_STREAM_RING) * S.k1 * S.slots * 2u : nullptr;
		A.prev_iq = S.prev_iq[S.parity0];
		A.dem_hist = S.dem[S.parity0];
		A.audio_host = (float *)ah;
		A.audio = S.audio_bufs[j & 3u];
#ifdef STREAM_TL
		const unsigned long long pt1 = __builtin_amdgcn_s_memtime();
		if (threadIdx.x == 0 && S.tl && !helper && p < 4u && j < 256u)
			S.tl[(7300u + j) * 8u + p * 2u] = __builtin_amdgcn_s_memrealtime();
#endif
		const bool drain = sh[5] != 0u;
		if (sh[7] != 0u) {
			A.run = S.drain_run;
			A.ntiles = S.drain_ntiles;
		}
		const unsigned int tasks_j = A.ntiles * A.groups;
		unsigned int mine = 0;
		const unsigned int rot = (unsigned int)(((unsigned long long)j * tasks) % S.n_post);
		for (unsigned int t = p >= rot ? p - rot : p + S.n_post - rot;; t += S.n_post) {
			if (drain) {
				if (threadIdx.x == 0)
					sh[4] = __hip_atomic_fetch_add(&S.sdev->post_ticket[j], 1u, __ATOMIC_RELAXED, __HIP_MEMORY_SCOPE_AGENT);
				__syncthreads();
				t = sh[4];
			}
			if (t >= tasks_j)
				break;
			post_role<D2, false, NSEG>(A, t % A.ntiles, t / A.ntiles, stage, tile, modes);
			__syncthreads();
			++mine;
		}
		if (threadIdx.x == 0 && mine) {
			if (ah)
				__builtin_amdgcn_fence(__ATOMIC_RELEASE, "");
			else
				__builtin_amdgcn_fence(__ATOMIC_RELEASE, "agent");
			asm volatile("s_waitcnt vmcnt(0)" ::: "memory");
			__hip_atomic_fetch_add(&S.sdev->post_done[j], mine, __ATOMIC_RELAXED, __HIP_MEMORY_SCOPE_AGENT);
		}
#ifdef STREAM_TL
		if (threadIdx.x == 0 && S.tl && !helper && p < 4u && j < 256u)
			S.tl[(7300u + j) * 8u + p * 2u + 1u] = __builtin_amdgcn_s_memrealtime();
		if (threadIdx.x == 0) {
			const unsigned long long pt3 = __builtin_amdgcn_s_memtime();
			pt_wait += pt1 - pt0;
			pt_sync += pt3 - pt1;
			++pt_n;
		}
#endif
	}
#ifdef STREAM_TL
	if (threadIdx.x == 0 && S.tl && !helper) {
		S.tl[(6000u + p) * 8u + 0u] = pt_wait;
		S.tl[(6000u + p) * 8u + 1u] = pt_sync;
		S.tl[(6000u + p) * 8u + 2u] = pt_n;
	}
#endif
	if (!helper && p < S.post.groups && known && known <= WR_STREAM_MAXJ) {
		const unsigned int jl = known - 1u;
		WrPostArgs A = S.post;
		A.chan_iq = S.ring + (size_t)(jl % WR_STREAM_RING) * S.k1 * S.slots * 2u;
		A.chan_prev = jl ? S.ring + (size_t)((jl - 1u) % WR_STREAM_RING) * S.k1 * S.slots * 2u : nullptr;
		A.prev_iq = S.prev_iq[S.parity0];
		A.dem_hist = S.dem[S.parity0];
		A.prev_next = const_cast<float *>(S.prev_iq[S.parity0 ^ 1]);
		A.dem_hist_next = S.dem[S.parity0 ^ 1];
		post_role<D2, false, NSEG>(A, A.ntiles, p, stage, tile, modes);
	}
}

template <unsigned int NG, unsigned int TS>
__device__ __forceinline__ void stream_ddc(const WrStreamArgs &S, v2f *lds)
{
	static_assert(TS == 1u || (TS == WR_TAPSETS && NG == 1u), "several channel filters: one lane group per wave");
	constexpr int NCO = WR_NCO_ROTATE;
	const unsigned int lane = threadIdx.x & 63u;
	const unsigned int wave = st_rfl(threadIdx.x >> 6);
	const unsigned int waves_per_wg = blockDim.x >> 6;
	const unsigned int wid = blockIdx.x * waves_per_wg + wave;
	wave_prio(3u);
	rot_tables_to_lds(lds, (const float2 *)S.hi_cs, (const float2 *)S.lo_cs);
	const v2f *hi_l = lds, *lo_l = lds + WR_SPLIT_N;
	const unsigned int nset = TS == 1u ? 1u : S.kmax;
	v2f *win = lds + 2u * WR_SPLIT_N + wave * (128u * nset);
	const unsigned int k1s = S.k1, d1 = S.d1;
	const unsigned int nwaves = S.n_ddc * waves_per_wg;
	const unsigned int gsets = S.groups / NG;
	const unsigned int wpg = nwaves / gsets;
	const unsigned int gs = wid % gsets;
	const unsigned int iw = wid / gsets;
	unsigned int known = 1;
	bool closed = false;
	if (iw < wpg) {
		const unsigned long long q0 = (unsigned long long)S.kslow + iw;
		LeanRec<NG> R = lean_rec<NG>([&](unsigned int s) { return S.phase[s]; }, S.step, S.flags, (const float4 *)S.rot,
		                             (float2 *)S.ring, S.gmap0, S.gmap1, gs, lane, (unsigned int)(q0 * d1 - WR_HIST), wpg, d1);
		const LeanWin<TS> W = lean_win<TS>(S.taps1u, S.tapsel, R.g0, lane, nset, win);
		unsigned int j = 0, k = (unsigned int)q0;
		while (k >= k1s) {
			k -= k1s;
			++j;
		}
		unsigned int jf = j, kf = k;
		unsigned int jb = 0xFFFFFFFFu;
		unsigned long long base_cur = 0, base_prev = 0;
		const bool u8 = S.is_u8 != 0u, ext = S.ext != 0u;
		unsigned int ahead = 0;
		bool drain = false;
		auto try_fetch = [&](float2 &dst) __attribute__((always_inline)) {
			if (drain)
				return;
			if (jf >= WR_STREAM_MAXJ) {
				drain = true;
				return;
			}
			if (jf >= known) {
				if (!closed) {
					const unsigned int r = st_ld(&S.sdev->ready);
					if (r > known)
						known = r;
					if (jf >= known && st_ld(&S.sdev->stop)) {
						const unsigned int f = st_ld(&S.sdev->ready);
						if (f > known)
							known = f;
						closed = true;
					}
				}
				if (jf >= known) {
					drain = true;
					return;
				}
			}
			if (jf != jb) {
				if (jf) {
					const unsigned long long a0 = __hip_atomic_load(&S.sdev->cur[jf], __ATOMIC_RELAXED, __HIP_MEMORY_SCOPE_AGENT);
					const unsigned long long a1 = __hip_atomic_load(&S.sdev->cur[jf + 1u], __ATOMIC_RELAXED, __HIP_MEMORY_SCOPE_AGENT);
					base_prev = ((unsigned long long)st_rfl((unsigned int)(a0 >> 32)) << 32) | st_rfl((unsigned int)a0);
					base_cur = ((unsigned long long)st_rfl((unsigned int)(a1 >> 32)) << 32) | st_rfl((unsigned int)a1);
				} else {
					base_prev = 0;
					base_cur = S.cur0;
				}
				jb = jf;
			}
			const long long n = (long long)kf * d1 - WR_HIST + lane;
			const unsigned long long base = (n >= 0) ? base_cur : base_prev;
			const unsigned long long idx = (n >= 0) ? (unsigned long long)n : (unsigned long long)((long long)S.nframes + n);
			if (ext) {
				if (u8) {
					const unsigned short b2 = __hip_atomic_load((const __attribute__((address_space(1))) unsigned short *)base + idx,
					                                            __ATOMIC_RELAXED, __HIP_MEMORY_SCOPE_AGENT);
					dst = make_float2(__builtin_bit_cast(float, (unsigned int)b2), 0.0f);
				} else {
					const unsigned long long x2 = __hip_atomic_load((const __attribute__((address_space(1))) unsigned long long *)base + idx,
					                                                __ATOMIC_RELAXED, __HIP_MEMORY_SCOPE_AGENT);
					dst = make_float2(__builtin_bit_cast(float, (unsigned int)x2), __builtin_bit_cast(float, (unsigned int)(x2 >> 32)));
				}
			} else if (u8) {
				const unsigned short b2 = ((const __attribute__((address_space(1))) unsigned short *)base)[idx];
				dst = make_float2(__builtin_bit_cast(float, (unsigned int)b2), 0.0f);
			} else {
				const v2f x2 = ((const __attribute__((address_space(1))) v2f *)base)[idx];
				dst = make_float2(x2.x, x2.y);
			}
			++ahead;
			kf += wpg;
			while (kf >= k1s) {
				kf -= k1s;
				++jf;
			}
		};
		unsigned int cnt = 0, pend_j = 0, pend_cnt = 0;
		unsigned int jring = 0xFFFFFFFFu;
		auto tell = [&]() __attribute__((always_inline)) {
			if (pend_cnt) {
				asm volatile("s_waitcnt vmcnt(0)" ::: "memory");
				if (lane == 0)
					__hip_atomic_fetch_add(&S.sdev->ddc_done[pend_j][wid % WR_STREAM_SHARDS][0], pend_cnt, __ATOMIC_RELAXED, __HIP_MEMORY_SCOPE_AGENT);
				pend_cnt = 0;
			}
		};
		static_assert(ROT_SEG == WR_FIR_LENGTH, "one recurrence over the whole window");
		float2 xa = make_float2(0.0f, 0.0f), xb = xa;
		unsigned long long tl_taps = 0, tl_rest = 0, tl_wait = 0, tl_units = 0, tl_ring = 0, tl_ringn = 0, tl_epochs = 0;
#ifdef STREAM_TL
		const bool tl_on = S.tl != nullptr;
#else
		constexpr bool tl_on = false;
#endif
		unsigned int lead = 0;
		auto unit = [&](float2 &xo, const int b) __attribute__((always_inline)) {
			const unsigned long long tl0 = tl_on ? __builtin_amdgcn_s_memtime() : 0ull;
			if (j != jring) {
				const unsigned long long pg = __hip_atomic_load(&S.sdev->progress, __ATOMIC_RELAXED, __HIP_MEMORY_SCOPE_AGENT);
				const unsigned int dr = st_rfl((unsigned int)pg), pr = st_rfl((unsigned int)(pg >> 32));
				lead = j > dr ? j - dr : 0u;
				if (j + 1u >= WR_STREAM_RING && pr < j - WR_STREAM_RING + 2u) {
					const unsigned long long tw0 = tl_on ? __builtin_amdgcn_s_memtime() : 0ull;
					tell();
					if (!stream_wait_count(S, (const unsigned int *)&S.sdev->progress + 1, j - WR_STREAM_RING + 2u)) {
						known = j;
						closed = true;
					}
					if (tl_on) {
						tl_ring += __builtin_amdgcn_s_memtime() - tw0;
						++tl_ringn;
#ifdef STREAM_TL
						if (lane == 0 && S.tl && (wid % 1000u) == 0u && j < 256u)
							S.tl[(7600u + j) * 8u + 4u + wid / 1000u] = __builtin_amdgcn_s_memrealtime();
#endif
					}
				}
				jring = j;
			}
			{
				wave_prio(lead <= 1u ? 2u : lead <= 3u ? 1u : 0u);
			}
			const AccN<NG> acc = rotate_unit<NG>(W.w4[b], R, S.table, hi_l, lo_l);
			const unsigned long long tl1 = tl_on ? __builtin_amdgcn_s_memtime() : 0ull;
			if (ahead >= 2u)
				W.to_lds(xo, b ^ 1, u8);
			unsigned long long tl2 = 0;
			if (tl_on) {
				asm volatile("s_waitcnt vmcnt(0) lgkmcnt(0)" ::: "memory");
				tl2 = __builtin_amdgcn_s_memtime();
			}
			tell();
			const size_t row = (size_t)(j % WR_STREAM_RING) * k1s + k;
#pragma unroll
			for (unsigned int c = 0; c < NG; ++c) {
				if (R.fl[c] & PHASE_FLAG_ACTIVE) {
					union { v2f f; unsigned long long u; } cv;
					cv.f = acc.v[c];
					__hip_atomic_store((unsigned long long *)&R.out[c][row * S.slots], cv.u, __ATOMIC_RELAXED,
					                   __HIP_MEMORY_SCOPE_AGENT);
				}
				R.Pk[c] += R.dP[c];
			}
			--ahead;
			cnt += NG;
			k += wpg;
			if (k >= k1s) {
				pend_j = j;
				pend_cnt = cnt;
				cnt = 0;
				do {
					k -= k1s;
					++j;
				} while (k >= k1s);
			}
			try_fetch(xo);
			if (tl_on) {
				const unsigned long long tl3 = __builtin_amdgcn_s_memtime();
				tl_taps += tl1 - tl0;
				tl_wait += tl2 - tl1;
				tl_rest += tl3 - tl2;
				++tl_units;
			}
		};
		for (;;) {
			if (j >= WR_STREAM_MAXJ || !stream_wait_ready(S, j, known, closed))
				break;
			drain = false;
			++tl_epochs;
			try_fetch(xa);
			try_fetch(xb);
			W.to_lds(xa, 0, u8);
			try_fetch(xa);
			wave_prio(2u);
			while (ahead) {
				unit(xb, 0);
				if (!ahead)
					break;
				unit(xa, 1);
			}
			wave_prio(3u);
			tell();
		}
		if (tl_on && lane == 0 && S.tl) {
			S.tl[wid * 8u + 0u] = tl_taps;
			S.tl[wid * 8u + 1u] = tl_wait;
			S.tl[wid * 8u + 2u] = tl_rest;
			S.tl[wid * 8u + 3u] = tl_units;
			S.tl[wid * 8u + 4u] = __builtin_amdgcn_s_getreg((31 << 11) | 4);
			S.tl[wid * 8u + 5u] = __builtin_amdgcn_s_getreg((31 << 11) | 20);
			S.tl[wid * 8u + 6u] = tl_ring;
			S.tl[wid * 8u + 7u] = (tl_ringn << 32) | tl_epochs;
		}
		asm volatile("s_waitcnt vmcnt(0)" ::: "memory");
		if (lane == 0) {
			if (pend_cnt)
				__hip_atomic_fetch_add(&S.sdev->ddc_done[pend_j][wid % WR_STREAM_SHARDS][0], pend_cnt, __ATOMIC_RELAXED, __HIP_MEMORY_SCOPE_AGENT);
			if (cnt && j < WR_STREAM_MAXJ)
				__hip_atomic_fetch_add(&S.sdev->ddc_done[j][wid % WR_STREAM_SHARDS][0], cnt, __ATOMIC_RELAXED, __HIP_MEMORY_SCOPE_AGENT);
		}
	}
	wave_prio(0u);
	(void)stream_wait_ready(S, 0xFFFFFFFEu, known, closed);
	const unsigned long long total = S.nframes * known;
	const unsigned int gtid = wid * 64u + lane, gsz = nwaves * 64u;
	const float *table = S.table;
	for (unsigned int s = gtid; s < S.slots; s += gsz) {
		const bool act = (S.flags[s] & PHASE_FLAG_ACTIVE) != 0;
		S.phase_next[s] = act ? S.phase[s] + (unsigned int)total * S.step[s] : S.phase[s];
	}
	for (unsigned int e = gtid; e < WR_HIST * S.slots; e += gsz) {
		const unsigned int r = e / S.slots, s = e - r * S.slots;
		const unsigned long long f = total + r;
		v2f cs = {0.0f, 0.0f}, lo = {0.0f, 0.0f};
		if (S.flags[s] & PHASE_FLAG_ACTIVE) {
			lo = nco<NCO>(S.phase[s] + (unsigned int)(f - WR_HIST) * S.step[s], table, hi_l, lo_l);
			cs = rot_into(S.phase[s], S.step[s], (unsigned int)(f - (WR_HIST - 1)), table);
		}
		((float2 *)S.hist_lo_next)[e] = make_float2(lo.x, lo.y);
		((float2 *)S.hist_cs_next)[e] = make_float2(cs.x, cs.y);
	}
	if (wid == 0 && known) {
		const unsigned long long c = known > 1u ? st_ld64(&S.sdev->desc[known - 1u].cur) : S.cur0;
		if (lane < WR_HIST) {
			const size_t n = (size_t)(S.nframes - WR_HIST + lane);
			float2 v;
			if (S.ext && S.is_u8) {
				const unsigned int b = __hip_atomic_load((const unsigned short *)c + n, __ATOMIC_RELAXED, __HIP_MEMORY_SCOPE_AGENT);
				v = make_float2(((float)(b & 255u) - 128.0f) / 128.0f, ((float)(b >> 8) - 128.0f) / 128.0f);
			} else if (S.ext) {
				const unsigned long long x = __hip_atomic_load((const unsigned long long *)c + n, __ATOMIC_RELAXED, __HIP_MEMORY_SCOPE_AGENT);
				v = make_float2(__builtin_bit_cast(float, (unsigned int)x), __builtin_bit_cast(float, (unsigned int)(x >> 32)));
			} else {
				v = input_frame(S.is_u8 ? nullptr : (const float2 *)c, S.is_u8 ? (const uchar2 *)c : nullptr, n);
			}
			((float2 *)S.hist_next)[lane] = v;
		}
		if (lane == 0)
			st_st_sys(&S.ctl->final_blocks, known);
	}
}

template <unsigned int PD2, unsigned int NG, unsigned int TS, unsigned int NSEG>
__global__ void __launch_bounds__(DDC_ROTATE_WAVES * 64u) __attribute__((amdgpu_waves_per_eu(DDC_NG2_WAVES_PER_EU)))
k_tuner_stream(const WrStreamArgs S)
{
	extern __shared__ v2f lds[];
	if (blockIdx.x >= S.n_ddc + S.n_post) {
		stream_bell(S);
		return;
	}
	const bool ddc = blockIdx.x < S.n_ddc;
	if (ddc) {
		stream_ddc<NG, TS>(S, lds);
		__syncthreads();
	}
	stream_post<PD2, TS, NSEG>(S, ddc ? blockIdx.x : blockIdx.x - S.n_ddc, lds, ddc);
}

static unsigned int stream_post_run(unsigned int tiles, unsigned int groups, unsigned int max_post)
{
	unsigned int run = 1;
	while (run < tiles && ((tiles + run - 1u) / run) * groups > max_post)
		++run;
	return run;
}

static size_t stream_lds_bytes(unsigned int d2, unsigned int nset, unsigned int nseg)
{
	const size_t post_lds = post_lds_bytes(d2, nseg) + 16u * sizeof(float);
	const size_t ddc_lds = (size_t)DDC_ROTATE_WAVES * 2u * 512u * nset + 2u * WR_SPLIT_N * 8u;
	return post_lds > ddc_lds ? post_lds : ddc_lds;
}

static void stream_shape(unsigned int groups, unsigned int kmax, bool one_filter, unsigned int *ng, unsigned int *ts)
{
	*ng = (one_filter && !(groups & 1u)) ? 2u : 1u;
	*ts = kmax > 1u ? WR_TAPSETS : 1u;
}

#define STREAM_NSEG4_MAX_D2 3u
static bool stream_nseg_supported(unsigned int d2, unsigned int nseg)
{
	return nseg == 1u || nseg == 2u || (nseg == 4u && d2 <= STREAM_NSEG4_MAX_D2);
}
template <unsigned int PD2, class F>
static hipError_t with_stream_nseg(unsigned int nseg, F &&f)
{
	if (nseg == 1u)
		return f(std::integral_constant<unsigned int, 1u>());
	if (nseg == 2u)
		return f(std::integral_constant<unsigned int, 2u>());
	if constexpr (PD2 <= STREAM_NSEG4_MAX_D2)
		if (nseg == 4u)
			return f(std::integral_constant<unsigned int, 4u>());
	return hipErrorInvalidValue;
}

template <unsigned int PD2, unsigned int NG, unsigned int TS, unsigned int NSEG>
static hipError_t stream_allow_lds(size_t lds)
{
	static bool attr_done[WR_MAX_DEVICES];
	if (lds <= 64 * 1024)
		return hipSuccess;
	return allow_lds((const void *)k_tuner_stream<PD2, NG, TS, NSEG>, stream_lds_bytes(PD2, TS, NSEG), attr_done);
}

template <unsigned int PD2, unsigned int NG, unsigned int TS, unsigned int NSEG>
static hipError_t stream_occupancy(size_t lds, int *per_cu)
{
	hipError_t e = stream_allow_lds<PD2, NG, TS, NSEG>(lds);
	if (e != hipSuccess)
		return e;
	return hipOccupancyMaxActiveBlocksPerMultiprocessor(per_cu, k_tuner_stream<PD2, NG, TS, NSEG>, (int)(DDC_ROTATE_WAVES * 64u), lds);
}

hipError_t wrk_stream_geometry(unsigned int d2, unsigned int groups, unsigned int kmax, bool one_filter, unsigned int nseg,
                               int num_cus, unsigned int *n_ddc, unsigned int *n_post)
{
	*n_ddc = *n_post = 0;
	if (!wrk_tuner_post_supported(d2) || !stream_nseg_supported(d2, nseg) || !groups || groups > 16u || !kmax ||
	    kmax > WR_TAPSETS)
		return hipSuccess;
	unsigned int ng, ts;
	stream_shape(groups, kmax, one_filter, &ng, &ts);
	const size_t lds = stream_lds_bytes(d2, ts == 1u ? 1u : kmax, nseg);
	int per_cu = 0;
	hipError_t e = with_post_d2(d2, [&](auto D2) {
		constexpr unsigned int PD2 = decltype(D2)::value;
		return with_stream_nseg<PD2>(nseg, [&](auto NS) {
			constexpr unsigned int NSEG = decltype(NS)::value;
			return ts != 1u ? stream_occupancy<PD2, 1, WR_TAPSETS, NSEG>(lds, &per_cu)
			       : ng == 1u ? stream_occupancy<PD2, 1, 1, NSEG>(lds, &per_cu)
			                  : stream_occupancy<PD2, 2, 1, NSEG>(lds, &per_cu);
		});
	});
	if (e != hipSuccess)
		return e;
	if (per_cu > 3)
		per_cu = 3;
	if (per_cu < 2)
		return hipSuccess;
	*n_ddc = (unsigned int)(per_cu - 1) * (unsigned int)num_cus;
	*n_post = (unsigned int)num_cus - 4u;
	return hipSuccess;
}

template <unsigned int PD2, unsigned int NG, unsigned int TS, unsigned int NSEG>
static hipError_t launch_stream(hipStream_t st, const WrStreamArgs &A, void *ev_start, void *ev_stop)
{
	const size_t lds = stream_lds_bytes(PD2, TS == 1u ? 1u : A.kmax, NSEG);
	hipError_t e = stream_allow_lds<PD2, NG, TS, NSEG>(lds);
	if (e != hipSuccess)
		return e;
	const unsigned int grid = A.n_ddc + A.n_post + 1u;
	if (ev_start || ev_stop) {
		hipExtLaunchKernelGGL((k_tuner_stream<PD2, NG, TS, NSEG>), dim3(grid), dim3(DDC_ROTATE_WAVES * 64u), (uint32_t)lds, st,
		                      (hipEvent_t)ev_start, (hipEvent_t)ev_stop, 0u, A);
		return hipGetLastError();
	}
	k_tuner_stream<PD2, NG, TS, NSEG><<<grid, DDC_ROTATE_WAVES * 64u, lds, st>>>(A);
	return hipGetLastError();
}

hipError_t wrk_tuner_stream(hipStream_t st, const WrStreamArgs &A0, void *ev_start, void *ev_stop)
{
	WrStreamArgs A = A0;
	if (!A.n_ddc || !A.n_post || !A.groups || A.groups > 16u || !A.k1)
		return hipErrorInvalidValue;
	const unsigned int min_run = stream_post_run(A.post.tiles, A.post.groups, A.n_post);
	A.post.run = min_run;
	if (min_run >= 2u && A.n_post >= 8u)
		A.post.run = stream_post_run(A.post.tiles, A.post.groups, A.n_post / 2u);
	while (A.post.run < 4u && A.post.run < A.post.tiles &&
	       ((A.post.tiles + A.post.run - 1u) / A.post.run) * A.post.groups > A.n_post / 4u &&
	       ((A.post.tiles + A.post.run - 1u) / A.post.run) * A.post.groups <= A.n_post / 2u)
		++A.post.run;
	A.post.ntiles = (A.post.tiles + A.post.run - 1u) / A.post.run;
	A.drain_run = min_run < A.post.run ? min_run : A.post.run;
	A.drain_ntiles = (A.post.tiles + A.drain_run - 1u) / A.drain_run;
	const unsigned int tasks = A.post.ntiles * A.post.groups;
	(void)tasks;
	if (!A.kmax || A.kmax > WR_TAPSETS)
		return hipErrorInvalidValue;
	unsigned int ng, ts;
	stream_shape(A.groups, A.kmax, A.one_filter != 0u, &ng, &ts);
	if ((size_t)A.n_ddc * DDC_ROTATE_WAVES < A.groups / ng)
		return hipErrorInvalidValue;
	if (A.k1 < WR_FIR_LENGTH * A.post.nseg)
		return hipErrorInvalidValue;
	return with_post_d2(A.post.d2, [&](auto D2) {
		constexpr unsigned int PD2 = decltype(D2)::value;
		return with_stream_nseg<PD2>(A.post.nseg, [&](auto NS) {
			constexpr unsigned int NSEG = decltype(NS)::value;
			return ts != 1u ? launch_stream<PD2, 1, WR_TAPSETS, NSEG>(st, A, ev_start, ev_stop)
			       : ng == 2u ? launch_stream<PD2, 2, 1, NSEG>(st, A, ev_start, ev_stop)
			                  : launch_stream<PD2, 1, 1, NSEG>(st, A, ev_start, ev_stop);
		});
	});
}
```

### webradio_amd/csrc/wr_tuner_stream.hip

```cpp
#include "wr_capi_internal.h"


static unsigned long long *g_stream_tl = nullptr;
extern "C" int wr_debug_stream_tl(unsigned long long *out, size_t n)
{
	if (!g_stream_tl)
		return 1;
	memcpy(out, g_stream_tl, n * sizeof(unsigned long long));
	return 0;
}

static std::mutex g_stream_mu;
static wr_tuner *g_stream_on[WR_MAX_DEVICES];

static void stream_raw_free(wr_tuner::Stream &s)
{
	for (uint8_t *&r : s.raw) {
		(void)hipFree(r);
		r = nullptr;
	}
	s.raw_cap = 0;
}

void wrc_stream_free(wr_tuner *t)
{
	wr_tuner::Stream &s = t->stream;
	(void)hipHostFree(s.ctl);
	(void)hipHostFree(s.desc);
	(void)hipFree(s.sdev);
	(void)hipFree(s.ring);
	stream_raw_free(s);
	if (s.raw_ev)
		(void)hipEventDestroy(s.raw_ev);
	s.raw_ev = nullptr;
	s.ctl = nullptr;
	s.desc = nullptr;
	s.sdev = nullptr;
	s.ring = nullptr;
	s.ring_floats = 0;
}

int wrc_stream_check(wr_tuner *t)
{
	wr_tuner::Stream &s = t->stream;
	if (!s.unchecked)
		return WR_OK;
	s.unchecked = false;
	s.long_blocks += s.ctl->long_blocks;
	s.ctl->long_blocks = 0;
	if (s.ctl->err)
		return wrc_fail(WR_ERR_HIP, "streaming launch: a wait inside the launch ran into its deadline (code %u)", s.ctl->err);
	if (s.ctl->final_blocks != s.count)
		return wrc_fail(WR_ERR_STATE, "streaming launch: %u blocks rung, %u processed%s", s.count, s.ctl->final_blocks,
		                s.ctl->self_closed ? " (the launch had closed itself: the doorbell was silent too long)" : "");
	return WR_OK;
}

bool wrc_stream_follows(const wr_tuner *t, size_t nframes, int where, bool u8)
{
	const wr_tuner::Stream &s = t->stream;
	if (!s.live || !s.enabled || where != WR_DEVICE || nframes != s.nframes || u8 != s.u8 || s.count >= WR_STREAM_MAXJ)
		return false;
	if (s.g->dirty)
		return false;
	const auto idle = std::chrono::steady_clock::now() - s.last_bell;
	return idle < std::chrono::milliseconds(WR_STREAM_STALE_MS);
}

int wrc_stream_bell(wr_tuner *t, const void *iq, bool behind_upload)
{
	wr_tuner::Stream &s = t->stream;
	const unsigned int j = s.count;
	const unsigned long long seq = t->submit_seq++;
	float *slot = wrc_stream_ring_entry(t, s.g, seq, s.k2, wrc_group_slots_used(s.g), j);
	s.desc[j].cur = (unsigned long long)(uintptr_t)iq;
	s.desc[j].audio_host = (unsigned long long)(uintptr_t)slot;
	s.desc[j].count = j + 1u;
	std::atomic_thread_fence(std::memory_order_release);
	if (behind_upload) {
		HIP_TRY(hipStreamWriteValue32(t->dev->up_stream, &s.sdev->ready_up, j + 1u, 0));
		s.up_pending = true;
	} else {
		if (s.up_pending) {
			HIP_TRY(hipStreamSynchronize(t->dev->up_stream));
			s.up_pending = false;
		}
		s.ctl->ready = j + 1u;
	}
	std::atomic_thread_fence(std::memory_order_seq_cst);
	s.count = j + 1u;
	++s.blocks;
	s.last_bell = std::chrono::steady_clock::now();
	return WR_OK;
}

int wrc_stream_open(wr_tuner *t, const void *iq, size_t nframes, bool u8, bool *took)
{
	*took = false;
	wr_tuner::Stream &s = t->stream;
	wr_dev *d = t->dev;
	if (t->nco_mode != WR_NCO_ROTATE || !t->defer_post || t->mark_launches || (t->keep_mask & (1u << WR_STAGE_DEMOD)))
		return WR_OK;
	Group *g = wrc_single_group(t);
	if (!g || g->l1 != WR_FIR_LENGTH || g->d1b || g->seek_pending || !wrk_tuner_post_supported(g->d2))
		return WR_OK;
	if (g->l2 != WR_FIR_LENGTH && g->l2 != 2u * WR_FIR_LENGTH && g->l2 != 4u * WR_FIR_LENGTH)
		return WR_OK;
	const unsigned int nseg = g->l2 / WR_FIR_LENGTH;
	if (nframes < (size_t)g->l2 * g->d1 || nframes % ((size_t)g->d1 * g->d2) || nframes / g->d1 > 0x3FFFFFFFu)
		return WR_OK;
	if (wrc_dev_bind(d))
		return WR_ERR_HIP;
	if (int rc = wrc_tuner_launch_held(t))
		return rc;
	if (g->dirty)
		if (int rc = wrc_group_upload(t, g))
			return rc;
	const unsigned int used = wrc_group_slots_used(g), groups = used / 64u;
	if (!groups || groups > 16u)
		return WR_OK;
	const unsigned long long used_mask = (1ull << groups) - 1ull;
	if ((g->fewsets_mask & used_mask) != used_mask)
		return WR_OK;
	unsigned int kmax = 1;
	for (unsigned int gi = 0; gi < groups; ++gi)
		if (g->nsets[gi] > kmax)
			kmax = g->nsets[gi];
	if (int rc = wrc_dev_settle_stream(d))
		return rc;
	{
		std::lock_guard<std::mutex> lk(g_stream_mu);
		if (d->device < 0 || d->device >= WR_MAX_DEVICES || (g_stream_on[d->device] && g_stream_on[d->device] != t))
			return WR_OK;
	}
	if (s.unchecked) {
		HIP_TRY(wrc_dev_stream_sync(d));
		if (int rc = wrc_stream_check(t))
			return rc;
	}
	if (g->post_pending)
		if (int rc = wrc_tuner_flush(t))
			return rc;
	const size_t k1 = nframes / g->d1, k2 = k1 / g->d2;
	unsigned int n_ddc = 0, n_post = 0;
	HIP_TRY(wrk_stream_geometry(g->d2, groups, kmax, g->one_filter, nseg, d->num_cus, &n_ddc, &n_post));
	if (!n_ddc || !n_post)
		return WR_OK;
	if (!s.ctl)
		HIP_TRY(hipHostMalloc((void **)&s.ctl, sizeof(WrStreamCtl), hipHostMallocMapped | hipHostMallocCoherent));
	if (!s.desc)
		HIP_TRY(hipHostMalloc((void **)&s.desc, sizeof(WrStreamDesc) * WR_STREAM_MAXJ, hipHostMallocMapped | hipHostMallocCoherent));
	if (!s.sdev)
		HIP_TRY(hipMalloc((void **)&s.sdev, sizeof(WrStreamDev)));
	const size_t ring_floats = (size_t)WR_STREAM_RING * k1 * g->slots * 2u;
	if (ring_floats > s.ring_floats) {
		HIP_TRY(wrc_dev_stream_sync(d));
		(void)hipFree(s.ring);
		s.ring = nullptr;
		s.ring_floats = 0;
		HIP_TRY(hipMalloc((void **)&s.ring, ring_floats * sizeof(float)));
		s.ring_floats = ring_floats;
	}
	void *ctl_dev = nullptr, *desc_dev = nullptr;
	HIP_TRY(hipHostGetDevicePointer(&ctl_dev, s.ctl, 0));
	HIP_TRY(hipHostGetDevicePointer(&desc_dev, s.desc, 0));
	hipStream_t st = d->stream;

	const WrTunerLaunch L = wrc_group_launch(t, g, u8 ? nullptr : (const float *)iq, u8 ? (const uint8_t *)iq : nullptr, nframes);

	WrStreamArgs A;
	memset(&A, 0, sizeof(A));
	A.ctl = (WrStreamCtl *)ctl_dev;
	A.desc_host = (const WrStreamDesc *)desc_dev;
	A.sdev = s.sdev;
	A.idle_ticks = (unsigned long long)WR_STREAM_IDLE_MS * 100000ull;
	A.wait_ticks = (unsigned long long)WR_STREAM_WAIT_MS * 100000ull;
	A.n_ddc = n_ddc;
	A.n_post = n_post;
	if (getenv("WR_STREAM_TL") && atoi(getenv("WR_STREAM_TL"))) {
		static unsigned long long *tlbuf = nullptr;
		if (!tlbuf)
			HIP_TRY(hipHostMalloc((void **)&tlbuf, 8192 * 8 * sizeof(unsigned long long), hipHostMallocMapped | hipHostMallocCoherent));
		memset(tlbuf, 0, 8192 * 8 * sizeof(unsigned long long));
		void *tld = nullptr;
		HIP_TRY(hipHostGetDevicePointer(&tld, tlbuf, 0));
		A.tl = (unsigned long long *)tld;
		g_stream_tl = tlbuf;
	}
	A.nframes = nframes;
	A.k1 = (unsigned int)k1;
	A.d1 = g->d1;
	A.is_u8 = u8 ? 1u : 0u;
	A.ext = s.ext ? 1u : 0u;
	A.slots = g->slots;
	A.groups = groups;
	for (unsigned int gi = 0; gi < groups; ++gi)
		(gi < 8u ? A.gmap0 : A.gmap1) |= (unsigned long long)gi << ((gi & 7u) * 8u);
	A.kslow = (WR_HIST + g->d1 - 1u) / g->d1;
	if (A.kslow > k1)
		A.kslow = (unsigned int)k1;
	A.hist = L.hist;
	A.hist_next = L.hist_next;
	A.phase = g->dev.phase[g->sp];
	A.step = g->dev.step;
	A.phase_next = g->dev.phase[g->sp ^ 1];
	A.hist_cs = g->dev.hist_cs[g->sp];
	A.hist_lo = g->dev.hist_lo[g->sp];
	A.hist_cs_next = g->dev.hist_cs[g->sp ^ 1];
	A.hist_lo_next = g->dev.hist_lo[g->sp ^ 1];
	A.flags = g->dev.flags;
	A.taps1 = g->dev.taps1;
	A.rot = g->dev.rot;
	A.taps1u = g->dev.taps1u;
	A.tapsel = g->dev.tapsel;
	A.table = d->table_turn;
	A.hi_cs = d->hi_cs;
	A.lo_cs = d->lo_cs;
	A.ring = s.ring;
	for (int i = 0; i < 4; ++i)
		A.audio_bufs[i] = g->dev.audio_set[(g->audio_cur + i) & 3];
	A.post = wrk_post_args(L, g->dev);
	A.post.host_stride = k2;
	A.prev_iq[0] = g->dev.prev_iq[0];
	A.prev_iq[1] = g->dev.prev_iq[1];
	A.dem[0] = g->dev.dem[0];
	A.dem[1] = g->dev.dem[1];
	A.parity0 = g->parity;
	A.kmax = kmax;
	A.one_filter = g->one_filter ? 1u : 0u;

	++s.gen;
	s.g = g;
	s.count = 0;
	s.nframes = nframes;
	s.u8 = u8;
	s.parity0 = g->parity;
	s.k1 = k1;
	s.k2 = k2;
	s.last_iq = nullptr;
	const unsigned long long seq = t->submit_seq++;
	float *slot = wrc_stream_ring_entry(t, g, seq, k2, used, 0);
	s.ctl->ready = 1;
	s.ctl->stop = 0;
	s.ctl->done = 0;
	s.ctl->final_blocks = 0;
	s.ctl->long_blocks = 0;
	s.ctl->err = 0;
	s.ctl->self_closed = 0;
	s.desc[0].cur = (unsigned long long)(uintptr_t)iq;
	s.desc[0].audio_host = (unsigned long long)(uintptr_t)slot;
	std::atomic_thread_fence(std::memory_order_seq_cst);
	if (s.ext) {
		HIP_TRY(hipMemsetAsync(s.sdev, 0, offsetof(WrStreamDev, ready_up), st));
		const size_t after = offsetof(WrStreamDev, ready_up) + sizeof(unsigned int);
		HIP_TRY(hipMemsetAsync((char *)s.sdev + after, 0, offsetof(WrStreamDev, desc) - after, st));
	} else {
		HIP_TRY(hipMemsetAsync(s.sdev, 0, offsetof(WrStreamDev, desc), st));
	}
	A.cur0 = s.desc[0].cur;
	A.audio0 = s.desc[0].audio_host;

	void *ev0 = nullptr, *ev1 = nullptr;
	if (t->profiling && !(t->ev_used & 1))
		if (int rc = wrc_prof_pair_begin(t, &ev0, &ev1))
			return rc;
	HIP_TRY(wrk_tuner_stream(st, A, ev0, ev1));
	if (ev0)
		wrc_prof_pair_stamped(t);
	s.live = true;
	s.count = 1;
	++s.blocks;
	s.last_bell = std::chrono::steady_clock::now();
	d->streaming = t;
	{
		std::lock_guard<std::mutex> lk(g_stream_mu);
		g_stream_on[d->device] = t;
	}
	*took = true;
	return WR_OK;
}

int wrc_stream_host_u8(wr_tuner *t, const uint8_t *bytes, size_t nframes, bool *took)
{
	*took = false;
	wr_tuner::Stream &s = t->stream;
	wr_dev *d = t->dev;
	if (wrc_dev_bind(d))
		return WR_ERR_HIP;
	if (!wrc_host_mapped(bytes))
		return WR_OK;
	const size_t need = nframes * 2;
	if (need <= WR_STREAM_HOST_MIN_BYTES)
		return WR_OK;
	const bool follows = s.live && s.ext && wrc_stream_follows(t, nframes, WR_DEVICE, true);
	if (need > s.raw_cap) {
		if (int rc = wrc_stream_close(t))
			return rc;
		HIP_TRY(wrc_dev_stream_sync(d));
		if (d->up_stream)
			HIP_TRY(hipStreamSynchronize(d->up_stream));
		stream_raw_free(s);
		for (uint8_t *&r : s.raw)
			HIP_TRY(hipMalloc((void **)&r, need));
		s.raw_cap = need;
	}
	const unsigned int slot = (unsigned int)(s.raw_next & 3u);
	const unsigned int through = s.raw_idx[slot] + 2u < s.count ? s.raw_idx[slot] + 2u : s.count;
	if ((s.live || s.unchecked) && s.raw_gen[slot] == s.gen && s.ctl->done < through) {
		const auto t0 = std::chrono::steady_clock::now();
		while (s.ctl->done < through && !s.ctl->err)
			if (std::chrono::steady_clock::now() - t0 > std::chrono::milliseconds(4 * WR_STREAM_WAIT_MS))
				return wrc_fail(WR_ERR_HIP, "streaming launch: block %u did not finish", s.raw_idx[slot] + 1u);
	}
	{
		std::lock_guard<std::mutex> up_guard(*d->upload_lock);
		if (int rc = wrc_dev_up_stream(d))
			return rc;
		HIP_TRY(hipMemcpyAsync(s.raw[slot], bytes, need, hipMemcpyHostToDevice, d->up_stream));
		if (int rc = wrc_upload_mark_locked(d, d->up_stream))
			return rc;
	}
	if (follows) {
		s.raw_gen[slot] = s.gen;
		s.raw_idx[slot] = s.count;
		++s.raw_next;
		++s.host_blocks;
		t->last_staging = 3;
		*took = true;
		return wrc_stream_bell(t, s.raw[slot], true);
	}
	if (int rc = wrc_stream_close(t))
		return rc;
	if (!s.raw_ev)
		HIP_TRY(hipEventCreateWithFlags(&s.raw_ev, hipEventDisableTiming));
	if (!s.sdev)
		HIP_TRY(hipMalloc((void **)&s.sdev, sizeof(WrStreamDev)));
	HIP_TRY(hipStreamWriteValue32(d->up_stream, &s.sdev->ready_up, 0u, 0));
	HIP_TRY(hipEventRecord(s.raw_ev, d->up_stream));
	HIP_TRY(hipStreamWaitEvent(d->stream, s.raw_ev, 0));
	s.ext = true;
	bool opened = false;
	if (int rc = wrc_stream_open(t, s.raw[slot], nframes, true, &opened))
		return rc;
	s.raw_gen[slot] = opened ? s.gen : 0;
	s.raw_idx[slot] = 0;
	++s.raw_next;
	*took = true;
	if (opened) {
		++s.host_blocks;
		t->last_staging = 3;
		return WR_OK;
	}
	s.ext = false;
	t->last_staging = 1;
	return wrc_tuner_submit_now(t, s.raw[slot], nframes, WR_DEVICE, true);
}

int wrc_stream_close(wr_tuner *t)
{
	wr_tuner::Stream &s = t->stream;
	if (!s.live)
		return WR_OK;
	if (s.up_pending) {
		HIP_TRY(hipStreamSynchronize(t->dev->up_stream));
		s.ctl->ready = s.count;
		s.up_pending = false;
	}
	std::atomic_thread_fence(std::memory_order_seq_cst);
	s.ctl->stop = 1;
	std::atomic_thread_fence(std::memory_order_seq_cst);
	s.live = false;
	s.unchecked = true;
	if (t->dev->streaming == t)
		t->dev->streaming = nullptr;
	{
		std::lock_guard<std::mutex> lk(g_stream_mu);
		if (g_stream_on[t->dev->device] == t)
			g_stream_on[t->dev->device] = nullptr;
	}
	Group *g = s.g;
	const unsigned int J = s.count;
	for (Group *x : t->groups)
		if (x != g)
			x->last_k1 = x->last_k2 = 0;
	g->sp ^= 1;
	g->last_parity = s.parity0;
	g->parity = s.parity0 ^ 1;
	g->last_k1 = s.k1;
	g->last_k2 = s.k2;
	g->last_demod_kept = false;
	s.last_iq = s.ring + (size_t)((J - 1u) % WR_STREAM_RING) * s.k1 * g->slots * 2u;
	g->audio_cur = (int)((g->audio_cur + (J - 1u)) & 3u);
	g->dev.audio = g->dev.audio_set[g->audio_cur];
	t->in_par ^= 1;
	wrc_advance_phases(t, (unsigned long long)s.nframes * J);
	t->submitted = true;
	return WR_OK;
}

extern "C" int wr_tuner_set_streaming(wr_tuner *t, int enable)
{
	if (!t)
		return wrc_fail(WR_ERR_ARG, "tuner is NULL");
	if (wrc_dev_bind(t->dev))
		return WR_ERR_HIP;
	if (int rc = wrc_tuner_launch_held(t))
		return rc;
	t->stream.enabled = enable != 0;
	t->stream.host_bytes = enable >= 2;
	return WR_OK;
}

extern "C" int wr_tuner_stream_info(wr_tuner *t, int *live, unsigned long long *launches, unsigned long long *blocks)
{
	if (!t)
		return wrc_fail(WR_ERR_ARG, "tuner is NULL");
	if (live)
		*live = t->stream.live ? 1 : 0;
	if (launches)
		*launches = t->stream.gen;
	if (blocks)
		*blocks = t->stream.blocks;
	return WR_OK;
}

extern "C" int wr_tuner_stream_long_blocks(wr_tuner *t, unsigned long long *blocks)
{
	if (!t || !blocks)
		return wrc_fail(WR_ERR_ARG, "wr_tuner_stream_long_blocks: bad argument");
	*blocks = t->stream.long_blocks;
	return WR_OK;
}

extern "C" int wr_tuner_stream_host_blocks(wr_tuner *t, unsigned long long *blocks)
{
	if (!t || !blocks)
		return wrc_fail(WR_ERR_ARG, "wr_tuner_stream_host_blocks: bad argument");
	*blocks = t->stream.host_blocks;
	return WR_OK;
}
```

### webradio_amd/device.py

```python
import ctypes as C

import numpy as np

from . import capi
from .capi import check, ptr


class Device:

    def __init__(self, index=0, stream=None):
        self.lib = capi.load()
        h = C.c_void_p()
        check(self.lib.wr_dev_open(C.byref(h), index, ptr(stream) if stream else None))
        self.h = h
        self.index = index

    def close(self):
        if self.h:
            self.lib.wr_dev_close(self.h)
            self.h = None

    def sync(self):
        check(self.lib.wr_dev_sync(self.h))

    def malloc(self, nbytes):
        p = C.c_void_p()
        check(self.lib.wr_dev_malloc(self.h, nbytes, C.byref(p)))
        return p.value

    def free(self, p):
        check(self.lib.wr_dev_free(self.h, C.c_void_p(p)))

    def upload(self, arr):
        arr = np.ascontiguousarray(arr)
        p = self.malloc(max(arr.nbytes, 4))
        check(self.lib.wr_dev_upload(self.h, C.c_void_p(p), ptr(arr), arr.nbytes))
        return p

    def download(self, p, count, dtype=np.float32):
        out = np.empty(count, dtype=dtype)
        check(self.lib.wr_dev_download(self.h, ptr(out), C.c_void_p(p), out.nbytes))
        return out

    def mix(self, iq, phase, phase_step):
        iq = np.ascontiguousarray(iq, dtype=np.float32)
        n = iq.size // 2
        din = self.upload(iq)
        dout = self.malloc(max(iq.nbytes, 4))
        ph = C.c_uint(phase)
        check(self.lib.wr_mix(self.h, C.c_void_p(din), C.c_void_p(dout), n, C.byref(ph), phase_step))
        out = self.download(dout, 2 * n)
        self.free(din)
        self.free(dout)
        return out, ph.value

    def fir_decimate(self, x, channels, decimation, coeff, history_dev):
        x = np.ascontiguousarray(x, dtype=np.float32)
        nframes = x.size // channels
        nout = (nframes // decimation) * channels
        din = self.upload(x)
        dout = self.malloc(max(nout * 4, 4))
        coeff = np.ascontiguousarray(coeff, dtype=np.float32)
        check(self.lib.wr_fir_decimate_n(self.h, C.c_void_p(din), nframes, channels, decimation, coeff.size,
                                         ptr(coeff), C.c_void_p(history_dev), C.c_void_p(dout)))
        out = self.download(dout, nout)
        self.free(din)
        self.free(dout)
        return out

    def demod(self, mode, iq, prev):
        iq = np.ascontiguousarray(iq, dtype=np.float32)
        n = iq.size // 2
        din = self.upload(iq)
        dout = self.malloc(max(n * 4, 4))
        prev = np.array(prev, dtype=np.float32)
        check(self.lib.wr_demod(self.h, mode, C.c_void_p(din), n, ptr(prev), C.c_void_p(dout)))
        out = self.download(dout, n)
        self.free(din)
        self.free(dout)
        return out, prev


class Tuner:

    def __init__(self, dev, input_rate, max_channels, max_block_frames, nco=capi.WR_NCO_ROTATE):
        self.dev = dev
        self.lib = dev.lib
        h = C.c_void_p()
        check(self.lib.wr_tuner_create(C.byref(h), dev.h, input_rate, max_channels, max_block_frames, nco))
        self.h = h
        self.input_rate = input_rate

    def destroy(self):
        if self.h:
            self.lib.wr_tuner_destroy(self.h)
            self.h = None

    def add_receiver(self, if_hz, chan_passband, chan_rate, mode, audio_passband, audio_rate, fir_lengths=None,
                     stage2=None):
        c = C.c_int()
        check(self.lib.wr_chan_add(self.h, C.byref(c)))
        ch = c.value
        check(self.lib.wr_chan_set_if(self.h, ch, if_hz))
        l1, l2 = fir_lengths if fir_lengths else (capi.WR_FIR_LENGTH, capi.WR_FIR_LENGTH)
        check(self.lib.wr_chan_set_filter_n(self.h, ch, 0, l1, chan_passband, chan_rate))
        if stage2:
            check(self.lib.wr_chan_set_filter_n(self.h, ch, 2, stage2[0], stage2[1], stage2[2]))
        check(self.lib.wr_chan_set_filter_n(self.h, ch, 1, l2, audio_passband, audio_rate))
        check(self.lib.wr_chan_set_mode(self.h, ch, mode))
        return ch

    def keep_stages(self, *stages):
        mask = 0
        for st in stages:
            mask |= 1 << st
        check(self.lib.wr_tuner_keep_stages(self.h, mask))

    def flush(self):
        check(self.lib.wr_tuner_flush(self.h))

    def blocks_per_launch(self, n):
        check(self.lib.wr_tuner_set_blocks_per_launch(self.h, n))

    def streaming(self, enable=True):
        check(self.lib.wr_tuner_set_streaming(self.h, int(enable) if enable is not True else 1))

    def stream_info(self):
        live, launches, blocks = C.c_int(), C.c_ulonglong(), C.c_ulonglong()
        check(self.lib.wr_tuner_stream_info(self.h, C.byref(live), C.byref(launches), C.byref(blocks)))
        return bool(live.value), launches.value, blocks.value

    def stream_host_blocks(self):
        n = C.c_ulonglong()
        check(self.lib.wr_tuner_stream_host_blocks(self.h, C.byref(n)))
        return n.value

    def stream_long_blocks(self):
        n = C.c_ulonglong()
        check(self.lib.wr_tuner_stream_long_blocks(self.h, C.byref(n)))
        return n.value

    def mark_launches(self, enable=True):
        check(self.lib.wr_tuner_mark_launches(self.h, 1 if enable else 0))

    def seek(self, frame):
        check(self.lib.wr_tuner_seek(self.h, C.c_ulonglong(frame)))

    def fetch_audio_all(self):
        stride, frames, slots = C.c_size_t(), C.c_size_t(), C.c_uint()
        self.lib.wr_tuner_fetch_audio_all(self.h, None, 0, C.byref(stride), C.byref(frames), C.byref(slots))
        out = np.empty(max(1, slots.value * frames.value), dtype=np.float32)
        check(self.lib.wr_tuner_fetch_audio_all(self.h, ptr(out), out.size, C.byref(stride), C.byref(frames),
                                                C.byref(slots)))
        return out[: slots.value * frames.value].reshape(slots.value, frames.value)

    def slot(self, ch):
        s = C.c_int()
        check(self.lib.wr_chan_slot(self.h, ch, C.byref(s)))
        return s.value

    def audio_ring(self, depth):
        check(self.lib.wr_tuner_audio_ring(self.h, depth))

    def ring_acquire(self):
        p = C.POINTER(C.c_float)()
        stride, frames, slots, seq = C.c_size_t(), C.c_size_t(), C.c_uint(), C.c_ulonglong()
        check(self.lib.wr_tuner_audio_ring_acquire(self.h, C.byref(p), C.byref(stride), C.byref(frames),
                                                   C.byref(slots), C.byref(seq)))
        n = slots.value * stride.value
        a = np.ctypeslib.as_array(p, shape=(n,)).copy() if n else np.zeros(0, np.float32)
        return a.reshape(slots.value, stride.value)[:, : frames.value], seq.value

    def ring_release(self):
        check(self.lib.wr_tuner_audio_ring_release(self.h))

    def ring_stats(self):
        q, o = C.c_uint(), C.c_ulonglong()
        check(self.lib.wr_tuner_audio_ring_stats(self.h, C.byref(q), C.byref(o)))
        return q.value, o.value

    def submit_count(self):
        n = C.c_ulonglong()
        check(self.lib.wr_tuner_submit_count(self.h, C.byref(n)))
        return n.value

    def remove_receiver(self, ch):
        check(self.lib.wr_chan_remove(self.h, ch))

    def set_if(self, ch, if_hz):
        check(self.lib.wr_chan_set_if(self.h, ch, if_hz))

    def set_af_gain(self, ch, gain_db):
        check(self.lib.wr_chan_set_af_gain(self.h, ch, C.c_float(gain_db)))

    def set_squelch(self, ch, threshold_dbfs, enable=True):
        check(self.lib.wr_chan_set_squelch(self.h, ch, C.c_float(threshold_dbfs), 1 if enable else 0))

    def set_mode(self, ch, mode):
        check(self.lib.wr_chan_set_mode(self.h, ch, mode))

    def set_filter(self, ch, stage, passband, out_rate):
        check(self.lib.wr_chan_set_filter(self.h, ch, stage, passband, out_rate))

    def submit_host(self, iq):
        iq = np.ascontiguousarray(iq, dtype=np.float32)
        check(self.lib.wr_tuner_submit(self.h, ptr(iq), iq.size // 2, capi.WR_HOST))
        self.dev.sync()

    def submit_device(self, dev_ptr, nframes):
        check(self.lib.wr_tuner_submit(self.h, ptr(dev_ptr), nframes, capi.WR_DEVICE))

    def submit_u8_host(self, raw):
        check(self.lib.wr_tuner_submit_u8(self.h, raw.ctypes.data_as(C.c_void_p), raw.size // 2, capi.WR_HOST))

    def last_staging(self):
        how = C.c_int()
        check(self.lib.wr_tuner_last_staging(self.h, C.byref(how)))
        return how.value

    def submit_u8_device(self, dev_ptr, nframes):
        check(self.lib.wr_tuner_submit_u8(self.h, ptr(dev_ptr), nframes, capi.WR_DEVICE))

    def fetch(self, ch, stage, capacity):
        out = np.empty(max(capacity, 1), dtype=np.float32)
        n = C.c_size_t()
        check(self.lib.wr_chan_fetch(self.h, ch, stage, ptr(out), capacity, C.byref(n)))
        return out[: n.value].copy()

    def state(self, ch):
        ph = C.c_uint()
        prev = np.zeros(2, dtype=np.float32)
        check(self.lib.wr_chan_get_state(self.h, ch, C.byref(ph), ptr(prev)))
        return ph.value, prev

    def set_state(self, ch, phase, prev=None):
        p = None if prev is None else np.ascontiguousarray(prev, dtype=np.float32)
        check(self.lib.wr_chan_set_state(self.h, ch, phase, ptr(p)))

    def profile(self, enable):
        check(self.lib.wr_tuner_profile(self.h, int(enable)))

    def profile_read(self):
        n = C.c_uint()
        ms = C.c_double()
        check(self.lib.wr_tuner_profile_read(self.h, C.byref(n), C.byref(ms)))
        return n.value, ms.value

    def audio_dev(self):
        a = C.c_void_p()
        stride = C.c_size_t()
        frames = C.c_size_t()
        check(self.lib.wr_tuner_audio_dev(self.h, C.byref(a), C.byref(stride), C.byref(frames)))
        return a.value, stride.value, frames.value


class Spectrum:

    def __init__(self, dev, fft_size, hop=0):
        self.dev = dev
        self.lib = dev.lib
        self.n = fft_size
        h = C.c_void_p()
        check(self.lib.wr_spectrum_create(C.byref(h), dev.h, fft_size, hop))
        self.h = h

    def destroy(self):
        if self.h:
            self.lib.wr_spectrum_destroy(self.h)
            self.h = None

    def push_host(self, iq):
        iq = np.ascontiguousarray(iq, dtype=np.float32)
        check(self.lib.wr_spectrum_push(self.h, ptr(iq), iq.size // 2, capi.WR_HOST))

    def push_device(self, dev_ptr, nframes):
        check(self.lib.wr_spectrum_push(self.h, ptr(dev_ptr), nframes, capi.WR_DEVICE))

    def get_db(self):
        out = np.empty(self.n, dtype=np.float32)
        check(self.lib.wr_spectrum_get_db(self.h, ptr(out)))
        return out

    def get_bins(self):
        out = np.empty(2 * self.n, dtype=np.float32)
        check(self.lib.wr_spectrum_get_bins(self.h, ptr(out)))
        return out

    def waterfall_row(self, width, hold=0):
        db = np.empty(width, dtype=np.float32)
        pal = np.empty(width, dtype=np.uint8)
        check(self.lib.wr_spectrum_get_waterfall_row(self.h, width, hold, ptr(db), ptr(pal)))
        return db, pal

    def frames_done(self):
        n = C.c_ulong()
        check(self.lib.wr_spectrum_frames_done(self.h, C.byref(n)))
        return n.value

    def lazy_info(self):
        a, b = C.c_ulonglong(), C.c_ulonglong()
        check(self.lib.wr_spectrum_lazy_info(self.h, C.byref(a), C.byref(b)))
        return a.value, b.value

    def batch_db(self, iq_dev, nframes_fft, db_dev):
        check(self.lib.wr_spectrum_batch_db(self.h, ptr(iq_dev), nframes_fft, ptr(db_dev)))


class Ring:

    @staticmethod
    def make_id():
        lib = capi.load()
        buf = (C.c_ubyte * lib.wr_ring_id_bytes())()
        check(lib.wr_ring_make_id(buf, len(buf)))
        return bytes(buf)

    @staticmethod
    def rccl_version():
        v = C.c_int()
        check(capi.load().wr_ring_version(C.byref(v)))
        return v.value

    def __init__(self, dev, id_bytes, rank, world):
        self.lib = capi.load()
        h = C.c_void_p()
        buf = (C.c_ubyte * len(id_bytes)).from_buffer_copy(id_bytes)
        check(self.lib.wr_ring_create(C.byref(h), dev.h, buf, len(id_bytes), rank, world))
        self.h, self.rank, self.world = h, rank, world

    def exchange(self, send_dev, recv_dev, nfloats):
        check(self.lib.wr_ring_exchange(self.h, ptr(send_dev), ptr(recv_dev), nfloats))

    def exchange_after(self, tuner, send_dev, recv_dev, nfloats):
        check(self.lib.wr_ring_exchange_after(self.h, tuner.h, ptr(send_dev), ptr(recv_dev), nfloats))

    def wait(self):
        check(self.lib.wr_ring_wait(self.h))

    def exchanges(self):
        n = C.c_ulonglong()
        check(self.lib.wr_ring_info(self.h, None, None, C.byref(n)))
        return n.value

    def destroy(self):
        if self.h:
            self.lib.wr_ring_destroy(self.h)
            self.h = None
```

Measured before the change: 124,600.

## Assign contiguous output runs to DDC waves and fuse demod into the streaming DDC

Each DDC wave in the persistent streaming kernel now processes a contiguous run of decimated outputs, where before it took outputs strided by the wave count. Because consecutive samples now sit in one wave, it can compute the FM/AM demod of each sample against the previous one and write it to a new demod ring. Run-edge samples go to a separate edge ring, and raw IQ stores are skipped when not needed. The post stage reads these precomputed demod rows instead of recomputing them from IQ. This targets redundant IQ traffic and demod work in post, at the cost of extra ring buffers, more complex indexing and edge handling, and a change in the DDC load and fetch pattern.

```diff
diff --git a/include/webradio_amd.h b/include/webradio_amd.h
--- a/include/webradio_amd.h
+++ b/include/webradio_amd.h
@@ -163,6 +163,7 @@
 #define WR_STREAM_MAX_BLOCKS 512u
 int wr_tuner_set_streaming(wr_tuner *tuner, int enable);
 int wr_tuner_stream_info(wr_tuner *tuner, int *live, unsigned long long *launches, unsigned long long *blocks);
+int wr_tuner_stream_geometry(wr_tuner *tuner, unsigned int *waves, unsigned int *run_frames);
 int wr_tuner_stream_host_blocks(wr_tuner *tuner, unsigned long long *blocks);
 int wr_tuner_stream_long_blocks(wr_tuner *tuner, unsigned long long *blocks);
 
diff --git a/webradio_amd/capi.py b/webradio_amd/capi.py
--- a/webradio_amd/capi.py
+++ b/webradio_amd/capi.py
@@ -70,6 +70,7 @@
     "wr_tuner_stream_info": (C.c_int, [_vp, C.POINTER(C.c_int), C.POINTER(C.c_ulonglong), C.POINTER(C.c_ulonglong)]),
     "wr_tuner_stream_host_blocks": (C.c_int, [_vp, C.POINTER(C.c_ulonglong)]),
     "wr_tuner_stream_long_blocks": (C.c_int, [_vp, C.POINTER(C.c_ulonglong)]),
+    "wr_tuner_stream_geometry": (C.c_int, [_vp, C.POINTER(C.c_uint), C.POINTER(C.c_uint)]),
     "wr_tuner_seek": (C.c_int, [_vp, C.c_ulonglong]),
     "wr_tuner_audio_ring": (C.c_int, [_vp, _u32]),
     "wr_tuner_audio_ring_acquire": (C.c_int, [_vp, C.POINTER(C.POINTER(C.c_float)), C.POINTER(C.c_size_t),
diff --git a/webradio_amd/csrc/wr_capi_internal.h b/webradio_amd/csrc/wr_capi_internal.h
--- a/webradio_amd/csrc/wr_capi_internal.h
+++ b/webradio_amd/csrc/wr_capi_internal.h
@@ -179,6 +179,10 @@
 		WrStreamDev *sdev = nullptr;
 		float *ring = nullptr;
 		size_t ring_floats = 0;
+		float *dem_ring = nullptr;
+		float *edge_ring = nullptr;
+		size_t dem_floats = 0, edge_floats = 0;
+		unsigned int wpg = 0, run_len = 0;
 		Group *g = nullptr;
 		unsigned int count = 0;
 		size_t nframes = 0;
diff --git a/webradio_amd/csrc/wr_internal.h b/webradio_amd/csrc/wr_internal.h
--- a/webradio_amd/csrc/wr_internal.h
+++ b/webradio_amd/csrc/wr_internal.h
@@ -121,6 +121,15 @@
 	size_t       host_stride;
 	unsigned int nseg = 1;
 	const float *chan_prev = nullptr;
+};
+struct WrPostRows {
+	const float *dem_rows = nullptr;
+	const float *dem_prev = nullptr;
+	const float *edge = nullptr;
+	const float *edge_prev = nullptr;
+	unsigned int run_len = 0;
+	unsigned int runs_pb = 0;
+	unsigned int kiq = 0, kiq_prev = 0;
 };
 long wrk_tune_ng2_min_passes(long value, bool set);
 hipError_t wrk_tuner_ddc(hipStream_t st, const WrTunerLaunch &L, const WrGroupDev &G,
@@ -206,6 +215,9 @@
 	const int          *tapsel;
 	const float        *table, *hi_cs, *lo_cs;
 	float              *ring;
+	float              *dem_ring;
+	float              *edge_ring;
+	unsigned int        run_len, runs_pb;
 	float              *audio_bufs[4];
 	WrPostArgs          post;
 	unsigned int        drain_run, drain_ntiles;
@@ -217,6 +229,8 @@
 #define WR_STREAM_ERR_WAIT   1u
 hipError_t wrk_stream_geometry(unsigned int d2, unsigned int groups, unsigned int kmax, bool one_filter, unsigned int nseg,
                                int num_cus, unsigned int *n_ddc, unsigned int *n_post);
+void wrk_stream_runs(unsigned int groups, unsigned int kmax, bool one_filter, unsigned int n_ddc, unsigned int k1,
+                     unsigned int *wpg, unsigned int *run_len, unsigned int *runs_pb);
 hipError_t wrk_tuner_stream(hipStream_t st, const WrStreamArgs &A, void *ev_start, void *ev_stop);
 
 struct WrFftPlan {
diff --git a/webradio_amd/csrc/wr_kernels.hip b/webradio_amd/csrc/wr_kernels.hip
--- a/webradio_amd/csrc/wr_kernels.hip
+++ b/webradio_amd/csrc/wr_kernels.hip
@@ -375,9 +375,35 @@
 	return demod_one(m, z.x, z.y, zp.x, zp.y);
 }
 
-template <unsigned int D2, bool HREGS, unsigned int NSEG = 1u>
+__device__ __forceinline__ float stream_dem_row(const WrPostArgs &A, const WrPostRows &X, const bool prev, const unsigned int k, const unsigned int run,
+                                                const unsigned int rem, const unsigned int s, const int m, const unsigned int hist)
+{
+	const unsigned int slots = A.slots;
+	if (!prev && k >= A.k1)
+		return 0.0f;
+	if (prev && !X.dem_prev)
+		return A.dem_hist[(size_t)(k - (A.k1 - hist)) * slots + s];
+	const float *__restrict__ dem = prev ? X.dem_prev : X.dem_rows;
+	const float2 *__restrict__ edge = (const float2 *)(prev ? X.edge_prev : X.edge);
+	const unsigned int kiq = prev ? X.kiq_prev : X.kiq;
+	if (k < kiq) {
+		const float2 *__restrict__ iq = (const float2 *)(prev ? A.chan_prev : A.chan_iq);
+		const float2 z = iq[(size_t)k * slots + s];
+		const float2 zp = k ? iq[(size_t)(k - 1u) * slots + s] : ((const float2 *)A.prev_iq)[s];
+		return demod_one(m, z.x, z.y, zp.x, zp.y);
+	}
+	if (rem == 0u) {
+		const float2 z = edge[(size_t)(run * 2u) * slots + s];
+		const float2 zp = k ? edge[(size_t)(run * 2u - 1u) * slots + s]
+		                    : ((const float2 *)X.edge_prev)[(size_t)(X.runs_pb * 2u - 1u) * slots + s];
+		return demod_one(m, z.x, z.y, zp.x, zp.y);
+	}
+	return dem[(size_t)k * slots + s];
+}
+
+template <unsigned int D2, bool HREGS, unsigned int NSEG = 1u, bool STREAM = false>
 __device__ __forceinline__ void post_role(const WrPostArgs &A, unsigned int bx, unsigned int g,
-                                          float *stage, float *tile, int *modes)
+                                          float *stage, float *tile, int *modes, const WrPostRows *rows = nullptr)
 {
 	constexpr unsigned int HIST = WR_FIR_LENGTH * NSEG - 1u;
 	constexpr unsigned int NEED = (POST_TK - 1u) * D2 + WR_FIR_LENGTH * NSEG;
@@ -399,6 +425,15 @@
 		if (m < 0)
 			return;
 		const size_t first = k1;
+		if constexpr (STREAM) {
+			for (unsigned int r = row; r < HIST; r += NROW) {
+				const unsigned int k = k1 - HIST + r, run = k / rows->run_len;
+				A.dem_hist_next[(size_t)r * slots + s] = stream_dem_row(A, *rows, false, k, run, k - run * rows->run_len, s, m, HIST);
+			}
+			if (row == 0)
+				((float2 *)A.prev_next)[s] = chan_iq[(size_t)(k1 - 1u) * slots + s];
+			return;
+		}
 #pragma unroll
 		for (unsigned int r = row; r < HIST; r += NROW)
 			A.dem_hist_next[(size_t)r * slots + s] = post_row(chan_iq, k1, slots, s, m, prev_iq, dem_hist, first + r, chan_prev, HIST);
@@ -446,7 +481,36 @@
 			const unsigned int per = (NEED - first + NROW - 1u) / NROW;
 			const unsigned int beg = first + row * per;
 			const unsigned int end = (beg + per < NEED) ? beg + per : NEED;
-			if (r0 > HIST && r0 + NEED <= (size_t)k1 + HIST) {
+			if constexpr (STREAM) {
+				const size_t rr0 = r0 + beg;
+				bool prev = rr0 < HIST;
+				unsigned int k = prev ? (unsigned int)(k1 - HIST + rr0) : (unsigned int)(rr0 - HIST);
+				const unsigned int run_len = rows->run_len;
+				unsigned int run = k / run_len, rem = k - run * run_len;
+				for (unsigned int r = beg; r < end; r += POST_LB) {
+					float v[POST_LB];
+#pragma unroll
+					for (unsigned int i = 0; i < POST_LB; ++i) {
+						v[i] = 0.0f;
+						if (r + i < end) {
+							v[i] = stream_dem_row(A, *rows, prev, k, run, rem, s, m, HIST);
+							++k;
+							if (++rem == run_len) {
+								rem = 0;
+								++run;
+							}
+							if (prev && k == k1) {
+								prev = false;
+								k = run = rem = 0;
+							}
+						}
+					}
+#pragma unroll
+					for (unsigned int i = 0; i < POST_LB; ++i)
+						if (r + i < end)
+							stage[(r + i) * 64u + lane] = (m >= 0) ? v[i] : 0.0f;
+				}
+			} else if (r0 > HIST && r0 + NEED <= (size_t)k1 + HIST) {
 				const float2 *__restrict__ src = chan_iq + (r0 - HIST) * slots + s;
 				for (unsigned int r = beg; r < end; r += POST_LB) {
 					float2 z[POST_LB + 1u];
diff --git a/webradio_amd/csrc/wr_stream_kernel.inc b/webradio_amd/csrc/wr_stream_kernel.inc
--- a/webradio_amd/csrc/wr_stream_kernel.inc
+++ b/webradio_amd/csrc/wr_stream_kernel.inc
@@ -237,6 +237,21 @@
 	}
 }
 
+__device__ __forceinline__ WrPostRows stream_post_rows(const WrStreamArgs &S, const unsigned int j)
+{
+	WrPostRows X;
+	const size_t dem_blk = (size_t)S.k1 * S.slots, edge_blk = (size_t)S.runs_pb * 2u * S.slots * 2u;
+	X.dem_rows = S.dem_ring + (size_t)(j % WR_STREAM_RING) * dem_blk;
+	X.edge = S.edge_ring + (size_t)(j % WR_STREAM_RING) * edge_blk;
+	X.dem_prev = j ? S.dem_ring + (size_t)((j - 1u) % WR_STREAM_RING) * dem_blk : nullptr;
+	X.edge_prev = j ? S.edge_ring + (size_t)((j - 1u) % WR_STREAM_RING) * edge_blk : nullptr;
+	X.run_len = S.run_len;
+	X.runs_pb = S.runs_pb;
+	X.kiq = j ? 0u : S.kslow + 1u;
+	X.kiq_prev = j == 1u ? S.kslow + 1u : 0u;
+	return X;
+}
+
 template <unsigned int PD2, unsigned int TS, unsigned int NSEG>
 __device__ __forceinline__ void stream_post(const WrStreamArgs &S, const unsigned int p, v2f *lds, const bool helper)
 {
@@ -344,6 +359,7 @@
 		WrPostArgs A = S.post;
 		A.chan_iq = S.ring + (size_t)(j % WR_STREAM_RING) * S.k1 * S.slots * 2u;
 		A.chan_prev = j ? S.ring + (size_t)((j - 1u) % WR_STREAM_RING) * S.k1 * S.slots * 2u : nullptr;
+		const WrPostRows X = stream_post_rows(S, j);
 		A.prev_iq = S.prev_iq[S.parity0];
 		A.dem_hist = S.dem[S.parity0];
 		A.audio_host = (float *)ah;
@@ -370,7 +386,7 @@
 			}
 			if (t >= tasks_j)
 				break;
-			post_role<D2, false, NSEG>(A, t % A.ntiles, t / A.ntiles, stage, tile, modes);
+			post_role<D2, false, NSEG, true>(A, t % A.ntiles, t / A.ntiles, stage, tile, modes, &X);
 			__syncthreads();
 			++mine;
 		}
@@ -405,11 +421,12 @@
 		WrPostArgs A = S.post;
 		A.chan_iq = S.ring + (size_t)(jl % WR_STREAM_RING) * S.k1 * S.slots * 2u;
 		A.chan_prev = jl ? S.ring + (size_t)((jl - 1u) % WR_STREAM_RING) * S.k1 * S.slots * 2u : nullptr;
+		const WrPostRows X = stream_post_rows(S, jl);
 		A.prev_iq = S.prev_iq[S.parity0];
 		A.dem_hist = S.dem[S.parity0];
 		A.prev_next = const_cast<float *>(S.prev_iq[S.parity0 ^ 1]);
 		A.dem_hist_next = S.dem[S.parity0 ^ 1];
-		post_role<D2, false, NSEG>(A, A.ntiles, p, stage, tile, modes);
+		post_role<D2, false, NSEG, true>(A, A.ntiles, p, stage, tile, modes, &X);
 	}
 }
 
@@ -436,16 +453,54 @@
 	unsigned int known = 1;
 	bool closed = false;
 	if (iw < wpg) {
-		const unsigned long long q0 = (unsigned long long)S.kslow + iw;
+		const unsigned int Rn = S.run_len, rpb = S.runs_pb;
+		struct RunPos {
+			unsigned int j, r, k, kend;
+		};
+		auto run_set = [&](RunPos &P) __attribute__((always_inline)) {
+			P.k = P.r * Rn;
+			P.kend = P.k + Rn < k1s ? P.k + Rn : k1s;
+		};
+		auto run_next = [&](RunPos &P) __attribute__((always_inline)) {
+			P.r += wpg;
+			do {
+				P.r -= rpb;
+				++P.j;
+			} while (P.r >= rpb);
+			run_set(P);
+		};
+		RunPos P;
+		P.j = 0;
+		P.r = iw;
+		while (P.r >= rpb) {
+			P.r -= rpb;
+			++P.j;
+		}
+		run_set(P);
+		if (P.j == 0u) {
+			if (P.k < S.kslow)
+				P.k = S.kslow;
+			if (P.k >= P.kend)
+				run_next(P);
+		}
+		RunPos F = P;
 		LeanRec<NG> R = lean_rec<NG>([&](unsigned int s) { return S.phase[s]; }, S.step, S.flags, (const float4 *)S.rot,
-		                             (float2 *)S.ring, S.gmap0, S.gmap1, gs, lane, (unsigned int)(q0 * d1 - WR_HIST), wpg, d1);
+		                             (float2 *)S.ring, S.gmap0, S.gmap1, gs, lane, (P.j * k1s + P.k) * d1 - WR_HIST, 1u, d1);
 		const LeanWin<TS> W = lean_win<TS>(S.taps1u, S.tapsel, R.g0, lane, nset, win);
-		unsigned int j = 0, k = (unsigned int)q0;
-		while (k >= k1s) {
-			k -= k1s;
-			++j;
-		}
-		unsigned int jf = j, kf = k;
+		unsigned int sl[NG];
+#pragma unroll
+		for (unsigned int c = 0; c < NG; ++c) {
+			const unsigned int gl = gs * NG + c;
+			sl[c] = (unsigned int)(((gl < 8u ? S.gmap0 : S.gmap1) >> ((gl & 7u) * 8u)) & 255u) * 64u + lane;
+			R.fl[c] = (R.fl[c] & PHASE_FLAG_ACTIVE) | (int)((unsigned int)S.post.mode[sl[c]] << 4);
+		}
+		v2f zp[NG];
+#pragma unroll
+		for (unsigned int c = 0; c < NG; ++c)
+			zp[c] = (v2f){0.0f, 0.0f};
+		bool havep = false;
+		bool store_iq = true;
+		const bool always_iq = S.post.squelch != nullptr;
 		unsigned int jb = 0xFFFFFFFFu;
 		unsigned long long base_cur = 0, base_prev = 0;
 		const bool u8 = S.is_u8 != 0u, ext = S.ext != 0u;
@@ -454,40 +509,40 @@
 		auto try_fetch = [&](float2 &dst) __attribute__((always_inline)) {
 			if (drain)
 				return;
-			if (jf >= WR_STREAM_MAXJ) {
+			if (F.j >= WR_STREAM_MAXJ) {
 				drain = true;
 				return;
 			}
-			if (jf >= known) {
+			if (F.j >= known) {
 				if (!closed) {
 					const unsigned int r = st_ld(&S.sdev->ready);
 					if (r > known)
 						known = r;
-					if (jf >= known && st_ld(&S.sdev->stop)) {
+					if (F.j >= known && st_ld(&S.sdev->stop)) {
 						const unsigned int f = st_ld(&S.sdev->ready);
 						if (f > known)
 							known = f;
 						closed = true;
 					}
 				}
-				if (jf >= known) {
+				if (F.j >= known) {
 					drain = true;
 					return;
 				}
 			}
-			if (jf != jb) {
-				if (jf) {
-					const unsigned long long a0 = __hip_atomic_load(&S.sdev->cur[jf], __ATOMIC_RELAXED, __HIP_MEMORY_SCOPE_AGENT);
-					const unsigned long long a1 = __hip_atomic_load(&S.sdev->cur[jf + 1u], __ATOMIC_RELAXED, __HIP_MEMORY_SCOPE_AGENT);
+			if (F.j != jb) {
+				if (F.j) {
+					const unsigned long long a0 = __hip_atomic_load(&S.sdev->cur[F.j], __ATOMIC_RELAXED, __HIP_MEMORY_SCOPE_AGENT);
+					const unsigned long long a1 = __hip_atomic_load(&S.sdev->cur[F.j + 1u], __ATOMIC_RELAXED, __HIP_MEMORY_SCOPE_AGENT);
 					base_prev = ((unsigned long long)st_rfl((unsigned int)(a0 >> 32)) << 32) | st_rfl((unsigned int)a0);
 					base_cur = ((unsigned long long)st_rfl((unsigned int)(a1 >> 32)) << 32) | st_rfl((unsigned int)a1);
 				} else {
 					base_prev = 0;
 					base_cur = S.cur0;
 				}
-				jb = jf;
-			}
-			const long long n = (long long)kf * d1 - WR_HIST + lane;
+				jb = F.j;
+			}
+			const long long n = (long long)F.k * d1 - WR_HIST + lane;
 			const unsigned long long base = (n >= 0) ? base_cur : base_prev;
 			const unsigned long long idx = (n >= 0) ? (unsigned long long)n : (unsigned long long)((long long)S.nframes + n);
 			if (ext) {
@@ -508,11 +563,8 @@
 				dst = make_float2(x2.x, x2.y);
 			}
 			++ahead;
-			kf += wpg;
-			while (kf >= k1s) {
-				kf -= k1s;
-				++jf;
-			}
+			if (++F.k >= F.kend)
+				run_next(F);
 		};
 		unsigned int cnt = 0, pend_j = 0, pend_cnt = 0;
 		unsigned int jring = 0xFFFFFFFFu;
@@ -535,27 +587,33 @@
 		unsigned int lead = 0;
 		auto unit = [&](float2 &xo, const int b) __attribute__((always_inline)) {
 			const unsigned long long tl0 = tl_on ? __builtin_amdgcn_s_memtime() : 0ull;
-			if (j != jring) {
+			if (P.j != jring) {
 				const unsigned long long pg = __hip_atomic_load(&S.sdev->progress, __ATOMIC_RELAXED, __HIP_MEMORY_SCOPE_AGENT);
 				const unsigned int dr = st_rfl((unsigned int)pg), pr = st_rfl((unsigned int)(pg >> 32));
-				lead = j > dr ? j - dr : 0u;
-				if (j + 1u >= WR_STREAM_RING && pr < j - WR_STREAM_RING + 2u) {
+				lead = P.j > dr ? P.j - dr : 0u;
+				if (P.j + 1u >= WR_STREAM_RING && pr < P.j - WR_STREAM_RING + 2u) {
 					const unsigned long long tw0 = tl_on ? __builtin_amdgcn_s_memtime() : 0ull;
 					tell();
-					if (!stream_wait_count(S, (const unsigned int *)&S.sdev->progress + 1, j - WR_STREAM_RING + 2u)) {
-						known = j;
+					if (!stream_wait_count(S, (const unsigned int *)&S.sdev->progress + 1, P.j - WR_STREAM_RING + 2u)) {
+						known = P.j;
 						closed = true;
 					}
 					if (tl_on) {
 						tl_ring += __builtin_amdgcn_s_memtime() - tw0;
 						++tl_ringn;
 #ifdef STREAM_TL
-						if (lane == 0 && S.tl && (wid % 1000u) == 0u && j < 256u)
-							S.tl[(7600u + j) * 8u + 4u + wid / 1000u] = __builtin_amdgcn_s_memrealtime();
+						if (lane == 0 && S.tl && (wid % 1000u) == 0u && P.j < 256u)
+							S.tl[(7600u + P.j) * 8u + 4u + wid / 1000u] = __builtin_amdgcn_s_memrealtime();
 #endif
 					}
 				}
-				jring = j;
+				jring = P.j;
+				if (!closed && known <= P.j + 1u) {
+					const unsigned int r = st_ld(&S.sdev->ready);
+					if (r > known)
+						known = r;
+				}
+				store_iq = always_iq || known <= P.j + 1u || (P.j == 0u && P.k <= S.kslow);
 			}
 			{
 				wave_prio(lead <= 1u ? 2u : lead <= 3u ? 1u : 0u);
@@ -570,28 +628,51 @@
 				tl2 = __builtin_amdgcn_s_memtime();
 			}
 			tell();
-			const size_t row = (size_t)(j % WR_STREAM_RING) * k1s + k;
+			const unsigned int jslot = P.j % WR_STREAM_RING;
+			const size_t row = (size_t)jslot * k1s + P.k;
+			const bool last = P.k + 1u == P.kend;
+			const size_t erow = ((size_t)jslot * rpb + P.r) * 2u;
 #pragma unroll
 			for (unsigned int c = 0; c < NG; ++c) {
 				if (R.fl[c] & PHASE_FLAG_ACTIVE) {
 					union { v2f f; unsigned long long u; } cv;
 					cv.f = acc.v[c];
-					__hip_atomic_store((unsigned long long *)&R.out[c][row * S.slots], cv.u, __ATOMIC_RELAXED,
-					                   __HIP_MEMORY_SCOPE_AGENT);
+					if (store_iq)
+						__hip_atomic_store((unsigned long long *)&R.out[c][row * S.slots], cv.u, __ATOMIC_RELAXED,
+						                   __HIP_MEMORY_SCOPE_AGENT);
+					if (havep) {
+						const float dv = demod_one(R.fl[c] >> 4, acc.v[c].x, acc.v[c].y, zp[c].x, zp[c].y);
+						__hip_atomic_store((unsigned int *)&S.dem_ring[row * S.slots + sl[c]], __builtin_bit_cast(unsigned int, dv),
+						                   __ATOMIC_RELAXED, __HIP_MEMORY_SCOPE_AGENT);
+					} else {
+						__hip_atomic_store((unsigned long long *)S.edge_ring + erow * S.slots + sl[c], cv.u, __ATOMIC_RELAXED,
+						                   __HIP_MEMORY_SCOPE_AGENT);
+					}
+					if (last)
+						__hip_atomic_store((unsigned long long *)S.edge_ring + (erow + 1u) * S.slots + sl[c], cv.u, __ATOMIC_RELAXED,
+						                   __HIP_MEMORY_SCOPE_AGENT);
 				}
-				R.Pk[c] += R.dP[c];
+				zp[c] = acc.v[c];
 			}
 			--ahead;
 			cnt += NG;
-			k += wpg;
-			if (k >= k1s) {
-				pend_j = j;
+			if (!last) {
+				++P.k;
+				havep = true;
+#pragma unroll
+				for (unsigned int c = 0; c < NG; ++c)
+					R.Pk[c] += R.dP[c];
+			} else {
+				pend_j = P.j;
 				pend_cnt = cnt;
 				cnt = 0;
-				do {
-					k -= k1s;
-					++j;
-				} while (k >= k1s);
+				const unsigned int q = P.j * k1s + P.k;
+				run_next(P);
+				havep = false;
+				const unsigned int dq = P.j * k1s + P.k - q;
+#pragma unroll
+				for (unsigned int c = 0; c < NG; ++c)
+					R.Pk[c] += dq * R.dP[c];
 			}
 			try_fetch(xo);
 			if (tl_on) {
@@ -603,7 +684,7 @@
 			}
 		};
 		for (;;) {
-			if (j >= WR_STREAM_MAXJ || !stream_wait_ready(S, j, known, closed))
+			if (P.j >= WR_STREAM_MAXJ || !stream_wait_ready(S, P.j, known, closed))
 				break;
 			drain = false;
 			++tl_epochs;
@@ -635,8 +716,8 @@
 		if (lane == 0) {
 			if (pend_cnt)
 				__hip_atomic_fetch_add(&S.sdev->ddc_done[pend_j][wid % WR_STREAM_SHARDS][0], pend_cnt, __ATOMIC_RELAXED, __HIP_MEMORY_SCOPE_AGENT);
-			if (cnt && j < WR_STREAM_MAXJ)
-				__hip_atomic_fetch_add(&S.sdev->ddc_done[j][wid % WR_STREAM_SHARDS][0], cnt, __ATOMIC_RELAXED, __HIP_MEMORY_SCOPE_AGENT);
+			if (cnt && P.j < WR_STREAM_MAXJ)
+				__hip_atomic_fetch_add(&S.sdev->ddc_done[P.j][wid % WR_STREAM_SHARDS][0], cnt, __ATOMIC_RELAXED, __HIP_MEMORY_SCOPE_AGENT);
 		}
 	}
 	wave_prio(0u);
@@ -716,6 +797,17 @@
 {
 	*ng = (one_filter && !(groups & 1u)) ? 2u : 1u;
 	*ts = kmax > 1u ? WR_TAPSETS : 1u;
+}
+
+void wrk_stream_runs(unsigned int groups, unsigned int kmax, bool one_filter, unsigned int n_ddc, unsigned int k1,
+                     unsigned int *wpg, unsigned int *run_len, unsigned int *runs_pb)
+{
+	unsigned int ng, ts;
+	stream_shape(groups, kmax, one_filter, &ng, &ts);
+	const unsigned int gsets = groups / ng;
+	*wpg = gsets ? n_ddc * DDC_ROTATE_WAVES / gsets : 0u;
+	*run_len = *wpg ? (k1 + *wpg - 1u) / *wpg : 0u;
+	*runs_pb = *run_len ? (k1 + *run_len - 1u) / *run_len : 0u;
 }
 
 #define STREAM_NSEG4_MAX_D2 3u
@@ -826,6 +918,10 @@
 	stream_shape(A.groups, A.kmax, A.one_filter != 0u, &ng, &ts);
 	if ((size_t)A.n_ddc * DDC_ROTATE_WAVES < A.groups / ng)
 		return hipErrorInvalidValue;
+	unsigned int wpg;
+	wrk_stream_runs(A.groups, A.kmax, A.one_filter != 0u, A.n_ddc, A.k1, &wpg, &A.run_len, &A.runs_pb);
+	if (!A.run_len || !A.dem_ring || !A.edge_ring)
+		return hipErrorInvalidValue;
 	if (A.k1 < WR_FIR_LENGTH * A.post.nseg)
 		return hipErrorInvalidValue;
 	return with_post_d2(A.post.d2, [&](auto D2) {
diff --git a/webradio_amd/csrc/wr_tuner_stream.hip b/webradio_amd/csrc/wr_tuner_stream.hip
--- a/webradio_amd/csrc/wr_tuner_stream.hip
+++ b/webradio_amd/csrc/wr_tuner_stream.hip
@@ -29,6 +29,8 @@
 	(void)hipHostFree(s.desc);
 	(void)hipFree(s.sdev);
 	(void)hipFree(s.ring);
+	(void)hipFree(s.dem_ring);
+	(void)hipFree(s.edge_ring);
 	stream_raw_free(s);
 	if (s.raw_ev)
 		(void)hipEventDestroy(s.raw_ev);
@@ -38,6 +40,8 @@
 	s.sdev = nullptr;
 	s.ring = nullptr;
 	s.ring_floats = 0;
+	s.dem_ring = s.edge_ring = nullptr;
+	s.dem_floats = s.edge_floats = 0;
 }
 
 int wrc_stream_check(wr_tuner *t)
@@ -161,6 +165,30 @@
 		HIP_TRY(hipMalloc((void **)&s.ring, ring_floats * sizeof(float)));
 		s.ring_floats = ring_floats;
 	}
+	unsigned int wpg = 0, run_len = 0, runs_pb = 0;
+	wrk_stream_runs(groups, kmax, g->one_filter, n_ddc, (unsigned int)k1, &wpg, &run_len, &runs_pb);
+	if (!run_len)
+		return WR_OK;
+	const size_t dem_floats = (size_t)WR_STREAM_RING * k1 * g->slots;
+	const size_t edge_floats = (size_t)WR_STREAM_RING * runs_pb * 2u * g->slots * 2u;
+	if (dem_floats > s.dem_floats) {
+		HIP_TRY(wrc_dev_stream_sync(d));
+		(void)hipFree(s.dem_ring);
+		s.dem_ring = nullptr;
+		s.dem_floats = 0;
+		HIP_TRY(hipMalloc((void **)&s.dem_ring, dem_floats * sizeof(float)));
+		s.dem_floats = dem_floats;
+	}
+	if (edge_floats > s.edge_floats) {
+		HIP_TRY(wrc_dev_stream_sync(d));
+		(void)hipFree(s.edge_ring);
+		s.edge_ring = nullptr;
+		s.edge_floats = 0;
+		HIP_TRY(hipMalloc((void **)&s.edge_ring, edge_floats * sizeof(float)));
+		s.edge_floats = edge_floats;
+	}
+	s.wpg = wpg;
+	s.run_len = run_len;
 	void *ctl_dev = nullptr, *desc_dev = nullptr;
 	HIP_TRY(hipHostGetDevicePointer(&ctl_dev, s.ctl, 0));
 	HIP_TRY(hipHostGetDevicePointer(&desc_dev, s.desc, 0));
@@ -217,6 +245,8 @@
 	A.hi_cs = d->hi_cs;
 	A.lo_cs = d->lo_cs;
 	A.ring = s.ring;
+	A.dem_ring = s.dem_ring;
+	A.edge_ring = s.edge_ring;
 	for (int i = 0; i < 4; ++i)
 		A.audio_bufs[i] = g->dev.audio_set[(g->audio_cur + i) & 3];
 	A.post = wrk_post_args(L, g->dev);
@@ -424,6 +454,17 @@
 	return WR_OK;
 }
 
+extern "C" int wr_tuner_stream_geometry(wr_tuner *t, unsigned int *waves, unsigned int *run_frames)
+{
+	if (!t)
+		return wrc_fail(WR_ERR_ARG, "tuner is NULL");
+	if (waves)
+		*waves = t->stream.wpg;
+	if (run_frames)
+		*run_frames = t->stream.run_len;
+	return WR_OK;
+}
+
 extern "C" int wr_tuner_stream_long_blocks(wr_tuner *t, unsigned long long *blocks)
 {
 	if (!t || !blocks)
diff --git a/webradio_amd/device.py b/webradio_amd/device.py
--- a/webradio_amd/device.py
+++ b/webradio_amd/device.py
@@ -130,6 +130,11 @@
         check(self.lib.wr_tuner_stream_info(self.h, C.byref(live), C.byref(launches), C.byref(blocks)))
         return bool(live.value), launches.value, blocks.value
 
+    def stream_geometry(self):
+        waves, run = C.c_uint(), C.c_uint()
+        check(self.lib.wr_tuner_stream_geometry(self.h, C.byref(waves), C.byref(run)))
+        return waves.value, run.value
+
     def stream_host_blocks(self):
         n = C.c_ulonglong()
         check(self.lib.wr_tuner_stream_host_blocks(self.h, C.byref(n)))
```

Measured after the change: 117,800. 0.946x the previous value.
